# yamrom/smash-paper

Hardware: AMD Instinct MI355X
Metric: reads/sec mapped+binned (hg19, 150 bp) at 1/2/4/8 MI355X; bit-exact bin counts (higher is better)
Workload: dtype u8/u64 (integer); 1 GPU; C3 hg19-shaped, 50 M x 150 bp SMASH reads per rank (25 M pairs, one run in batches), sample_bins/50000; genome=hg19, index_words=packed (SA / ISA hints, DESIGN section 3), genome_bp=3095693983, text_N=6191388016, pairs_per_rank=25000000, read_len=150, batch_pairs=12500000, bins=50000, parallelism=single GPU

## Files before the change

smash-paper_amd/csrc/keyset.hpp:

```cpp
#pragma once

namespace smash {
namespace {

constexpr int kRefShift = 40;
constexpr uint64_t kRefPub = 1ull << 39;
struct KeyRef {
  const uint64_t *w;
  uint32_t nk;
  uint64_t lo;
};

__device__ bool same_key(const uint64_t *rec, const KeyRef &k) {
  if (rec[0] != k.lo || rec[1] != k.nk) return false;
  for (uint32_t i = 0; i < k.nk; ++i)
    if (rec[2 + i] != k.w[i]) return false;
  return true;
}

__device__ bool same_key(const KeyRef &a, const KeyRef &b) {
  if (a.lo != b.lo || a.nk != b.nk) return false;
  for (uint32_t i = 0; i < a.nk; ++i)
    if (a.w[i] != b.w[i]) return false;
  return true;
}

__device__ inline void key_hashes(const uint64_t *w, uint32_t nk, uint64_t mask, uint64_t &hh,
                                  uint64_t &hl) {
  hh = 0x9E3779B97F4A7C15ull;
  hl = 0xD1B54A32D192ED03ull;
  for (uint32_t i = 0; i < nk; ++i) {
    const uint64_t x = w[i];
    hh = mix64(hh ^ x) + 0x632BE59BD9B4E019ull;
    hl = mix64(hl + x * 0x9E3779B97F4A7C15ull) ^ (hl >> 29);
  }
  hh = (mix64(hh ^ uint64_t(nk)) & mask) | 1;
  hl = (mix64(hl + uint64_t(nk)) & mask) | 1;
}

__host__ __device__ __forceinline__ uint64_t key_home(uint64_t hi, uint64_t mask) {
  return (hi ^ (hi >> 31)) & mask;
}

__device__ __forceinline__ uint32_t wave_incl(uint32_t v, uint32_t &total) {
  const uint32_t lane = threadIdx.x & 63;
#pragma unroll
  for (int d = 1; d < 64; d <<= 1) {
    const uint32_t y = __shfl_up(v, d, 64);
    if (lane >= uint32_t(d)) v += y;
  }
  total = __shfl(v, 63, 64);
  return v;
}

__device__ __forceinline__ uint32_t wave_word_owner(uint32_t incl, uint32_t t, uint32_t &before) {
  uint32_t l = 0;
#pragma unroll
  for (uint32_t step = 32; step; step >>= 1)
    if (uint32_t(__shfl(int(incl), int(l + step - 1), 64)) <= t) l += step;
  l = l < 63u ? l : 63u;
  const uint32_t prev = uint32_t(__shfl(int(incl), int((l + 63u) & 63u), 64));
  before = l ? prev : 0u;
  return l;
}

constexpr uint32_t kDecGroups = 4;

__device__ __forceinline__ void wave_fill_records(uint64_t *arena, uint64_t off, uint32_t incl,
                                                  uint32_t total, bool ok, uint64_t lo, uint32_t m,
                                                  const uint64_t *src) {
  const uint32_t lane = threadIdx.x & 63;
  const uint64_t srcv = reinterpret_cast<uint64_t>(src);
  for (uint32_t t0 = 0; t0 < total; t0 += 64) {
    const uint32_t t = t0 + lane;
    uint32_t before;
    const uint32_t l = wave_word_owner(incl, t, before);
    const uint32_t r = t - before;
    const bool lok = __shfl(int(ok), int(l), 64) != 0;
    const uint64_t loff = __shfl(off, int(l), 64), llo = __shfl(lo, int(l), 64);
    const uint32_t lm = uint32_t(__shfl(int(m), int(l), 64));
    const uint64_t *ls = reinterpret_cast<const uint64_t *>(__shfl(srcv, int(l), 64));
    if (t < total && lok) arena[loff + r] = r == 0 ? llo : r == 1 ? uint64_t(lm) : ls[r - 2];
  }
}

constexpr uint64_t kSlotOld = ~0ull, kSlotNone = ~0ull - 1;
constexpr uint64_t kSlotIns = 1ull << 62;

struct PairKeys {
  static constexpr bool kMarks = true;
  const int32_t *nk;
  const uint64_t *hash;
  HitRows hits;
  uint8_t *contest;
  __device__ __forceinline__ int32_t count(uint64_t q) const { return nk[q]; }
  __device__ __forceinline__ KeyRef key(uint64_t q, uint64_t *hi = nullptr) const {
    if (hi) *hi = hash[2 * q];
    const int32_t k = nk[q];
    return KeyRef{hits.row(q, k), uint32_t(k), hash[2 * q + 1]};
  }
};

struct RecvKeys {
  static constexpr bool kMarks = false;
  const uint64_t *recv, *words, *base;
  int world;
  uint64_t hmask;
  __device__ __forceinline__ int32_t count(uint64_t j) const {
    return int32_t(recv[kHdrWords * j] >> 40);
  }
  __device__ __forceinline__ KeyRef key(uint64_t j, uint64_t *hi = nullptr) const {
    int r = 0;
    while (r + 1 < world && j >= base[r + 1]) ++r;
    const uint64_t nw = recv[kHdrWords * j];
    KeyRef k{words + base[65 + r] + (nw & kHdrOffMask), uint32_t(nw >> 40), 0};
    uint64_t h = 0;
    key_hashes(k.w, k.nk, hmask, h, k.lo);
    if (hi) *hi = h;
    return k;
  }
};

template <class Src>
__device__ __forceinline__ uint64_t claim_key(const Src &src, uint64_t j, uint64_t *table,
                                              uint64_t mask, const uint64_t *arena,
                                              uint64_t epoch, int32_t &err) {
  uint64_t hi = 0;
  const KeyRef me = src.key(j, &hi);
  const unsigned long long mine = (epoch << kRefShift) | (j + 1);
  uint64_t res = kSlotNone;
  uint64_t i = key_home(hi, mask);
  uint32_t waits = 0;
  for (uint64_t probe = 0; probe <= mask;) {
    unsigned long long *sh = reinterpret_cast<unsigned long long *>(&table[2 * i]);
    unsigned long long *sr = sh + 1;
    unsigned long long cur = __hip_atomic_load(sh, __ATOMIC_RELAXED, __HIP_MEMORY_SCOPE_AGENT);
    if (cur == 0) {
      const unsigned long long prev = atomicCAS(sh, 0ull, (unsigned long long)hi);
      if (prev == 0) {
        __hip_atomic_store(sr, mine, __ATOMIC_RELAXED, __HIP_MEMORY_SCOPE_AGENT);
        res = Src::kMarks ? i | kSlotIns : i;
        break;
      }
      cur = prev;
    }
    if (cur == hi) {
      const unsigned long long ref =
          __hip_atomic_load(sr, __ATOMIC_RELAXED, __HIP_MEMORY_SCOPE_AGENT);
      if (ref == 0) {
        if (++waits > (1u << 22)) {
          err = SMASH_ERR_UNSUPPORTED;
          break;
        }
        continue;
      }
      if (ref & kRefPub) {
        if ((ref >> kRefShift) != epoch &&
            same_key(arena + ((ref & (kRefPub - 1)) - 1), me)) {
          res = kSlotOld;
          break;
        }
      } else if ((ref >> kRefShift) == epoch) {
        const uint64_t j2 = (ref & (kRefPub - 1)) - 1;
        if (same_key(me, src.key(j2))) {
          if constexpr (Src::kMarks) src.contest[j2] = 1;
          atomicMin(sr, mine);
          res = i;
          break;
        }
      }
    }
    ++probe;
    i = (i + 1) & mask;
  }
  if (res == kSlotNone && err == 0) err = SMASH_ERR_NOMEM;
  return res;
}

template <class Src, class Item>
__device__ __forceinline__ bool decide_keys(const Src &src, uint64_t n, uint64_t *table,
                                            uint64_t *arena, uint64_t arena_cap,
                                            unsigned long long *arena_top, uint64_t epoch,
                                            const uint64_t *__restrict__ slot_of, Item item) {
  const uint64_t stride = uint64_t(gridDim.x) * blockDim.x;
  bool full = false;
  const uint32_t lane = threadIdx.x & 63;
  for (uint64_t c0 = (uint64_t(blockIdx.x) * blockDim.x + (threadIdx.x & ~63u)) * kDecGroups;
       c0 < n; c0 += stride * kDecGroups) {
    bool wins[kDecGroups];
    uint32_t needs[kDecGroups], incls[kDecGroups], tots[kDecGroups];
    uint32_t sum = 0;
#pragma unroll
    for (uint32_t g = 0; g < kDecGroups; ++g) {
      const uint64_t j = c0 + 64 * g + lane;
      const int32_t m = j < n ? src.count(j) : -1;
      bool win = false;
      if (m >= 0) {
        const uint64_t sl = slot_of[j];
        bool sole = false;
        if constexpr (Src::kMarks) sole = sl < kSlotNone && (sl & kSlotIns) && !src.contest[j];
        if (sole) {
          win = true;
        } else if (sl < kSlotNone) {
          const unsigned long long ref = __hip_atomic_load(
              reinterpret_cast<unsigned long long *>(&table[2 * (sl & ~kSlotIns) + 1]),
              __ATOMIC_RELAXED, __HIP_MEMORY_SCOPE_AGENT);
          win = ref == ((epoch << kRefShift) | (j + 1));
        }
      }
      wins[g] = win;
      needs[g] = win ? 2u + uint32_t(m) : 0u;
      incls[g] = wave_incl(needs[g], tots[g]);
      sum += tots[g];
    }
    unsigned long long wbase = 0;
    if (lane == 63 && sum) wbase = atomicAdd(arena_top, (unsigned long long)sum);
    wbase = __shfl(wbase, 63, 64);
#pragma unroll
    for (uint32_t g = 0; g < kDecGroups; ++g) {
      const uint64_t j = c0 + 64 * g + lane;
      const bool win = wins[g];
      const uint32_t need = needs[g], incl = incls[g], total = tots[g];
      const uint64_t off = uint64_t(wbase) + incl - need;
      wbase += total;
      const bool ok = win && off + need <= arena_cap;
      KeyRef me{nullptr, 0u, 0ull};
      if (win) me = src.key(j);
      wave_fill_records(arena, off, incl, total, ok, me.lo, me.nk, me.w);
      if (win) {
        if (!ok) {
          full = true;
        } else {
          __hip_atomic_store(
              reinterpret_cast<unsigned long long *>(&table[2 * (slot_of[j] & ~kSlotIns) + 1]),
              (unsigned long long)((epoch << kRefShift) | kRefPub | (off + 1)), __ATOMIC_RELAXED,
              __HIP_MEMORY_SCOPE_AGENT);
        }
      }
      if (j < n) item(j, win);
    }
  }
  return full;
}

__global__ void k_dedup_claim(const int32_t *__restrict__ nk, const uint64_t *__restrict__ hash,
                              HitRows hits, uint64_t n,
                              uint64_t *table, uint64_t mask, const uint64_t *arena,
                              uint64_t epoch, uint64_t *slot_of, uint8_t *contest,
                              unsigned long long *stats) {
  SMASH_BESIDE_SEARCH();
  const PairKeys src{nk, hash, hits, contest};
  const uint64_t stride = uint64_t(gridDim.x) * blockDim.x;
  int32_t err = 0;
  for (uint64_t q = uint64_t(blockIdx.x) * blockDim.x + threadIdx.x; q < n; q += stride)
    if (nk[q] >= 0) slot_of[q] = claim_key(src, q, table, mask, arena, epoch, err);
  if (err) atomicCAS(&stats[S_ERR], 0ull, (unsigned long long)(unsigned)err);
}

__global__ void k_dedup_decide(const int32_t *__restrict__ nk, const uint64_t *__restrict__ hash,
                               HitRows hits,
                               const uint32_t *__restrict__ nmajor,
                               const int64_t *__restrict__ chrom_off, uint64_t n,
                               uint64_t *table, uint64_t *arena, uint64_t arena_cap,
                               unsigned long long *arena_top, uint64_t epoch,
                               const uint64_t *__restrict__ slot_of,
                               const uint8_t *__restrict__ contest, uint8_t *keep,
                               uint32_t *cnt, int64_t *lp, unsigned long long *stats) {
  SMASH_BESIDE_SEARCH();
  const PairKeys src{nk, hash, hits, const_cast<uint8_t *>(contest)};
  unsigned long long kp = 0, dp = 0;
  const bool full = decide_keys(
      src, n, table, arena, arena_cap, arena_top, epoch, slot_of,
      [&](uint64_t q, bool win) __attribute__((always_inline)) {
        const int32_t m = nk[q];
        if (m >= 0) {
          ++kp;
          dp += win ? 0 : 1;
        }
        keep[q] = win ? 1 : 0;
        const uint32_t c = win ? nmajor[q] : 0;
        cnt[q] = c;
        int64_t last = -1;
        if (c) {
          const uint64_t *h = hits.row(q, m);
          for (int32_t j = m - 1; j >= 0; --j)
            if (chrom_off[uint32_t(h[j] >> 48)] >= 0) {
              last = int64_t(h[j] & 0xFFFFFFFFFFFFull);
              break;
            }
        }
        lp[q] = last;
      });
  wave_stats(stats, S_KEYPAIRS, kp, S_DUPEPAIRS, dp, full ? SMASH_ERR_NOMEM : 0);
}

__global__ void k_owner_claim(const uint64_t *recv, const uint64_t *words, const uint64_t *base,
                              int world, uint64_t n, uint64_t *table, uint64_t mask,
                              const uint64_t *arena, uint64_t epoch, uint64_t *slot_of,
                              unsigned long long *stats, uint64_t hmask) {
  const RecvKeys src{recv, words, base, world, hmask};
  const uint64_t stride = uint64_t(gridDim.x) * blockDim.x;
  int32_t err = 0;
  for (uint64_t j = uint64_t(blockIdx.x) * blockDim.x + threadIdx.x; j < n; j += stride)
    slot_of[j] = claim_key(src, j, table, mask, arena, epoch, err);
  if (err) atomicCAS(&stats[S_ERR], 0ull, (unsigned long long)(unsigned)err);
}

__global__ void k_owner_decide(const uint64_t *recv, const uint64_t *words, const uint64_t *base,
                               int world, uint64_t n, uint64_t *table, uint64_t *arena,
                               uint64_t arena_cap, unsigned long long *arena_top, uint64_t epoch,
                               const uint64_t *__restrict__ slot_of, uint8_t *flags,
                               unsigned long long *stats, uint64_t hmask) {
  const RecvKeys src{recv, words, base, world, hmask};
  const bool full = decide_keys(src, n, table, arena, arena_cap, arena_top, epoch, slot_of,
                                [&](uint64_t j, bool win) __attribute__((always_inline)) {
                                  flags[j] = win ? 1 : 0;
                                });
  if (full) atomicCAS(&stats[S_ERR], 0ull, (unsigned long long)(unsigned)SMASH_ERR_NOMEM);
}

}
}

static void key_set_geometry(uint64_t keys, uint64_t max_pairs, uint64_t *slots,
                             uint64_t *arena_words) {
  const uint64_t cap = 2 * std::max<uint64_t>(keys, max_pairs);
  uint64_t pw = 1;
  while (pw < cap) pw <<= 1;
  *slots = pw;
  *arena_words = std::min<uint64_t>(16 * std::max<uint64_t>(keys, max_pairs) + (1u << 20),
                                    smash::kRefPub - 2);
}

static uint64_t next_epoch(smash_pipeline *p) {
  p->epoch = p->epoch % ((1ull << (64 - smash::kRefShift)) - 1) + 1;
  return p->epoch;
}

__global__ void k_rehash(const uint64_t *__restrict__ old, uint64_t old_slots, uint64_t *nt,
                         uint64_t mask) {
  const uint64_t stride = uint64_t(gridDim.x) * blockDim.x;
  for (uint64_t i = uint64_t(blockIdx.x) * blockDim.x + threadIdx.x; i < old_slots; i += stride) {
    const uint64_t hi = old[2 * i];
    if (!hi) continue;
    uint64_t j = smash::key_home(hi, mask);
    for (uint64_t probe = 0; probe <= mask; ++probe, j = (j + 1) & mask) {
      unsigned long long *sh = reinterpret_cast<unsigned long long *>(&nt[2 * j]);
      if (atomicCAS(sh, 0ull, (unsigned long long)hi) == 0ull) {
        nt[2 * j + 1] = old[2 * i + 1];
        break;
      }
    }
  }
}
```

smash-paper_amd/csrc/pipeline.hip:

```cpp
#include <hipcub/hipcub.hpp>

#include <algorithm>
#include <cstdlib>
#include <cstring>

#include "common.hpp"
#include "mam_device.hpp"

namespace {
constexpr int kB = 256;
constexpr unsigned kPostBlocks = 64;
constexpr unsigned kPostThreads = kPostBlocks * kB;
enum Stat { S_PAIRS, S_KEYPAIRS, S_DUPEPAIRS, S_POS, S_DUPS, S_KEPT, S_MATCHES, S_ERR, S_N };
constexpr uint32_t kStatStride = 16, kStatStripes = 16, kStatWords = kStatStride * kStatStripes;
constexpr uint32_t kHdrWords = 1;
constexpr uint64_t kHdrOffMask = (uint64_t(1) << 40) - 1;
static_assert(kHdrWords == SMASH_EXPORT_HDR_WORDS, "smash_gpu.h's export header");
}

#define SMASH_BESIDE_SEARCH() __builtin_amdgcn_s_setprio(2)

struct smash_pipeline {
  const smash_index *ix = nullptr;
  int device = 0;
  uint32_t read_len = 0, min_len = 20, slots = 0, n_contig = 0, nbins = 0;
  uint32_t stride = 0;
  int32_t min_excess = 4;
  int64_t hit_window = 10000;
  uint64_t max_pairs = 0;
  uint32_t *d_tag_off = nullptr;
  uint8_t *d_small = nullptr;
  int64_t *d_chrom_off = nullptr;
  int64_t *d_bins = nullptr;
  uint32_t *d_cell = nullptr;
  uint32_t ncell = 0, cshift = 0;
  uint32_t *d_sp_cell = nullptr;
  uint32_t sp_ncell = 0, sp_shift = 0;
  uint64_t *d_match = nullptr;
  uint32_t *d_nmatch = nullptr;
  uint64_t *d_match_s[2] = {nullptr, nullptr};
  uint32_t *d_nmatch_s[2] = {nullptr, nullptr};
  uint8_t *d_rec_s[2] = {nullptr, nullptr};
  unsigned long long *d_work_s[2] = {nullptr, nullptr};
  uint64_t rec_bytes = 0;
  bool var_len = false;
  uint16_t *d_len_s[2] = {nullptr, nullptr};
  const uint16_t *d_lens = nullptr;
  hipStream_t xs[2] = {nullptr, nullptr};
  hipEvent_t ev_in = nullptr, ev_found[2] = {nullptr, nullptr}, ev_free[2] = {nullptr, nullptr};
  hipEvent_t ev_done = nullptr;
  bool set_used[2] = {false, false};
  bool defer_free = false;
  const uint8_t *pref_reads[2] = {nullptr, nullptr};
  uint64_t pref_n[2] = {0, 0};
  bool searched[2] = {false, false};
  int set = 1;
  int32_t *d_nk = nullptr;
  uint32_t *d_nmajor = nullptr;
  uint64_t *d_hits = nullptr;
  uint64_t *d_hhead = nullptr;
  uint64_t *d_hash = nullptr;
  uint8_t *d_keep = nullptr;
  uint64_t *d_slot = nullptr;
  uint8_t *d_contest = nullptr;
  uint64_t *d_tsum = nullptr;
  int64_t *d_tlast = nullptr;
  bool cnt_ready = false;
  bool reads_resident = false;
  uint64_t *d_bcnt = nullptr, *d_boff = nullptr;
  void *d_scan_temp = nullptr;
  size_t scan_temp_bytes = 0;
  uint64_t *d_oslot = nullptr;
  uint64_t oslot_cap = 0;
  uint64_t *d_table = nullptr;
  uint64_t table_mask = 0;
  uint64_t *d_arena = nullptr;
  uint64_t arena_cap = 0;
  unsigned long long *d_arena_top = nullptr;
  uint64_t keys_bound = 0;
  uint64_t epoch = 0;
  uint32_t *d_posoff = nullptr;
  uint32_t *d_cnt = nullptr;
  int64_t *d_pos0 = nullptr, *d_abs = nullptr;
  int64_t *d_prev = nullptr;
  int64_t *d_lp = nullptr, *d_lps = nullptr;
  uint32_t bin_flush = 0x8000;
  uint32_t *d_binpart = nullptr;
  bool bin_lds = true;
  bool pos_dirty = false;
  unsigned long long *d_stats = nullptr;
  uint32_t *d_fb = nullptr;
  uint32_t *d_l16 = nullptr;
  uint8_t *d_post_ws = nullptr;
  uint64_t hash_mask = ~0ull;
  bool post_fast = false;
  bool mhint = false;
  uint32_t post_cap = 0;
  uint32_t *d_send_q = nullptr;
  unsigned long long *d_owner = nullptr;
  uint64_t *d_send_hdr = nullptr;
  uint64_t *d_send_words = nullptr;
  uint64_t send_words_cap = 0;
  uint64_t *d_recv_base = nullptr;
  unsigned long long *h_owner = nullptr;
  uint64_t *h_recv_base = nullptr;
  hipEvent_t ev_base = nullptr;
  uint64_t n_pairs = 0, n_export = 0;
  hipStream_t last = nullptr;
  void *feed = nullptr;
  void (*feed_free)(void *) = nullptr;
  bool prof = false;
  std::vector<hipEvent_t> ev;
  uint64_t n_ev = 0, prof_reads = 0;
};

namespace smash {
namespace {

struct PostCfg {
  const uint64_t *startpos, *sizes;
  uint32_t n_seq, L, slots;
  const uint32_t *tag_off;
  const uint8_t *small;
  const int64_t *chrom_off;
  const uint8_t *map;
  uint64_t map_bytes;
  int32_t min_excess;
  int64_t window;
  uint32_t fast_cap;
  uint64_t hash_mask;
  const uint32_t *sp_cell;
  uint32_t sp_shift, sp_ncell;
  bool mhint;
  const uint16_t *lens;
};

constexpr uint64_t kRefMask = kPkPosMask;

constexpr uint32_t kHitHead = 16;
struct HitRows {
  uint64_t *head, *full;
  uint32_t slots;
  __device__ __forceinline__ uint64_t *row(uint64_t q, int32_t nk) const {
    return nk <= int32_t(kHitHead) ? head + q * kHitHead : full + q * 2 * uint64_t(slots);
  }
};

struct Aln {
  int64_t pos, qpos;
  uint32_t seq;
  uint16_t prefix, len, suffix;
  uint8_t rc, pad;
};

struct Hit {
  int64_t pos;
  uint32_t tid, qstart, qend;
  int32_t L0, R0;
  int64_t qkey;
  uint8_t rc;
};

__device__ inline bool merge_less(const Aln &a, const Aln &b) {
  if (a.rc != b.rc) return a.rc < b.rc;
  if (a.seq != b.seq) return a.seq < b.seq;
  if (a.pos != b.pos) return a.pos < b.pos;
  return a.prefix < b.prefix;
}

__device__ inline unsigned mapb(const PostCfg &c, uint64_t at) {
  return at < c.map_bytes ? c.map[at] : 0u;
}

template <bool VAR>
__device__ int mate_hits(const PostCfg &c, const uint64_t *m, uint32_t n,
                         Hit *hits, Aln *a, int32_t &err, uint32_t Lm) {
  int na = 0;
  const uint32_t L = VAR ? Lm : c.L;
  for (uint32_t k = 0; k < n; ++k) {
    const uint64_t w = m[k];
    const uint64_t ref = w & (c.mhint ? kRefMask : 0xFFFFFFFFFFFFull);
    const uint32_t q = uint32_t((w >> 48) & 0xFF), len = uint32_t(w >> 56);
    uint32_t lo = 0, hi = c.n_seq;
    while (lo < hi) {
      const uint32_t mid = (lo + hi) >> 1;
      if (c.startpos[mid] <= ref) lo = mid + 1; else hi = mid;
    }
    const uint32_t si = lo - 1;
    const uint64_t rcpos = ref - q;
    int64_t pos = int64_t(rcpos - c.startpos[si]);
    const uint32_t extra = L - len - q;
    Aln x;
    x.qpos = q;
    x.len = uint16_t(len);
    if (si & 1) {
      x.seq = si - 1;
      pos = int64_t(c.sizes[si - 1] - uint64_t(pos)) - int64_t(L);
      x.prefix = uint16_t(extra);
      x.suffix = uint16_t(q);
      x.rc = 1;
    } else {
      x.seq = si;
      x.prefix = uint16_t(q);
      x.suffix = uint16_t(extra);
      x.rc = 0;
    }
    x.pos = pos;
    if (pos >= 0) a[na++] = x;
  }
  for (int i = 1; i < na; ++i) {
    Aln t = a[i];
    int j = i - 1;
    while (j >= 0 && merge_less(t, a[j])) { a[j + 1] = a[j]; --j; }
    a[j + 1] = t;
  }
  int nh = 0;
  int g0 = 0;
  for (int i = 0; i < na; ++i) {
    const bool endg = (i + 1 == na) || a[i + 1].pos != a[i].pos ||
                      a[i + 1].seq != a[i].seq || a[i + 1].rc != a[i].rc;
    if (!endg) continue;
    Hit h;
    h.tid = a[i].seq >> 1;
    h.rc = a[i].rc;
    h.pos = a[i].pos;
    h.qstart = a[g0].prefix;
    h.qend = L - a[i].suffix;
    int64_t qmin = a[g0].qpos;
    for (int k = g0 + 1; k <= i; ++k) qmin = a[k].qpos < qmin ? a[k].qpos : qmin;
    h.qkey = qmin;
    const uint32_t abspos = c.tag_off[h.tid] + uint32_t(h.pos + 1);
    const bool small = c.small[h.tid] != 0;
    for (int k = g0; k <= i; ++k) {
      const uint32_t cnt = a[k].len;
      const uint32_t li = abspos + uint32_t(a[k].prefix) + cnt - 1;
      const uint32_t ri = abspos + uint32_t(a[k].prefix) - 1;
      const unsigned lm = mapb(c, 2 + uint64_t(li) * 2);
      const unsigned left = lm ? lm - 1 : 255;
      const unsigned rm = mapb(c, 2 + uint64_t(ri) * 2 + 1);
      const unsigned right = rm ? rm : 255;
      if (k == g0) { h.L0 = int32_t(left); h.R0 = int32_t(right); }
      if (!small && err == 0) {
        if (left > cnt) err = SMASH_ERR_TAG_LEFT;
        else if (right > cnt) err = SMASH_ERR_TAG_RIGHT;
      }
    }
    int j = nh - 1;
    while (j >= 0 && (h.qkey < hits[j].qkey || (h.qkey == hits[j].qkey && h.rc < hits[j].rc))) {
      hits[j + 1] = hits[j];
      --j;
    }
    hits[j + 1] = h;
    ++nh;
    g0 = i + 1;
  }
  return nh;
}

__device__ inline uint64_t mix64(uint64_t z) {
  z ^= z >> 33; z *= 0xff51afd7ed558ccdull;
  z ^= z >> 33; z *= 0xc4ceb9fe1a85ec53ull;
  z ^= z >> 33;
  return z;
}

__host__ __device__ inline uint64_t post_ws_bytes(uint32_t slots) {
  return (uint64_t(slots) * sizeof(Aln) + 2ull * slots * sizeof(Hit) + 15) & ~uint64_t(15);
}

template <bool VAR>
__device__ __noinline__ void post_pair(const PostCfg &c, const uint64_t *__restrict__ match,
                                       const uint32_t *__restrict__ nmatch, uint64_t q,
                                       int32_t *nk_out, uint32_t *nmajor_out,
                                       HitRows hits_out, uint64_t *hash_out, int32_t &err,
                                       unsigned long long &nm, uint8_t *ws) {
  {
    Aln *a = reinterpret_cast<Aln *>(ws);
    Hit *h1 = reinterpret_cast<Hit *>(ws + uint64_t(c.slots) * sizeof(Aln));
    Hit *h2 = h1 + c.slots;
    const uint32_t n1 = nmatch[2 * q], n2 = nmatch[2 * q + 1];
    nm = n1 + n2;
    const uint32_t L1 = VAR ? c.lens[2 * q] : 0u, L2 = VAR ? c.lens[2 * q + 1] : 0u;
    const int k1 = mate_hits<VAR>(c, match + (2 * q) * c.slots, n1 < c.slots ? n1 : c.slots, h1, a,
                                  err, L1);
    const int k2 = mate_hits<VAR>(c, match + (2 * q + 1) * c.slots, n2 < c.slots ? n2 : c.slots, h2,
                                  a, err, L2);
    if (n1 > c.slots || n2 > c.slots) err = SMASH_ERR_UNSUPPORTED;
    int m1 = 0, m2 = 0;
    for (int i = 0; i < k1; ++i) {
      const int mx = h1[i].L0 > h1[i].R0 ? h1[i].L0 : h1[i].R0;
      if (int(h1[i].qend) - int(h1[i].qstart) - mx >= c.min_excess) h1[m1++] = h1[i];
    }
    for (int i = 0; i < k2; ++i) {
      const int mx = h2[i].L0 > h2[i].R0 ? h2[i].L0 : h2[i].R0;
      if (int(h2[i].qend) - int(h2[i].qstart) - mx >= c.min_excess) h2[m2++] = h2[i];
    }
    uint64_t *ho = hits_out.full + q * (2 * uint64_t(c.slots));
    int32_t nk = -1;
    uint32_t nmaj = 0;
    uint64_t hh = 0x9E3779B97F4A7C15ull, hl = 0xD1B54A32D192ED03ull;
    if (m1 > 0 || m2 > 0) {
      nk = 0;
      auto put = [&](uint32_t tid, int64_t pos) {
        ho[nk++] = (uint64_t(tid) << 48) | (uint64_t(pos) & 0xFFFFFFFFFFFFull);
        const uint64_t w = (uint64_t(tid) << 48) ^ uint64_t(pos);
        hh = mix64(hh ^ w) + 0x632BE59BD9B4E019ull;
        hl = mix64(hl + w * 0x9E3779B97F4A7C15ull) ^ (hl >> 29);
        if (c.chrom_off[tid] >= 0) ++nmaj;
      };
      for (int i = 0; i < m1; ++i) put(h1[i].tid, h1[i].pos);
      for (int b = 0; b < m2; ++b) {
        bool close = false;
        for (int i = 0; i < m1; ++i) {
          int64_t d = h1[i].pos - h2[b].pos;
          d = d < 0 ? -d : d;
          if (h1[i].tid == h2[b].tid && d < c.window) { close = true; break; }
        }
        if (!close) put(h2[b].tid, h2[b].pos);
      }
      hh = (mix64(hh ^ uint64_t(nk)) & c.hash_mask) | 1;
      hl = (mix64(hl + uint64_t(nk)) & c.hash_mask) | 1;
      if (nk <= int32_t(kHitHead))
        for (int32_t i = 0; i < nk; ++i) hits_out.head[q * kHitHead + i] = ho[i];
    }
    nk_out[q] = nk;
    nmajor_out[q] = nmaj;
    hash_out[2 * q] = hh;
    hash_out[2 * q + 1] = hl;
  }
}

__device__ __forceinline__ unsigned long long wave_sum(unsigned long long v) {
#pragma unroll
  for (int d = 32; d >= 1; d >>= 1) v += __shfl_xor(v, d, 64);
  return v;
}

__device__ __forceinline__ unsigned long long *stat_row(unsigned long long *stats) {
  const uint32_t w = blockIdx.x * (blockDim.x / 64) + threadIdx.x / 64;
  return stats + kStatStride * (w % kStatStripes);
}

__device__ __forceinline__ void wave_stats(unsigned long long *stats, int ia,
                                           unsigned long long a, int ib, unsigned long long b,
                                           int32_t err) {
  a = wave_sum(a);
  b = wave_sum(b);
  unsigned long long *row = stat_row(stats);
  if ((threadIdx.x & 63) == 0) {
    if (a) atomicAdd(&row[ia], a);
    if (b) atomicAdd(&row[ib], b);
  }
  if (err) atomicCAS(&stats[S_ERR], 0ull, (unsigned long long)(unsigned)err);
}

__device__ __forceinline__ void post_stats(unsigned long long nm, unsigned long long np,
                                           int32_t err, unsigned long long *stats) {
  wave_stats(stats, S_MATCHES, nm, S_PAIRS, np, err);
}

template <bool VAR>
__global__ __launch_bounds__(kB) void k_post(PostCfg c, const uint64_t *__restrict__ match,
                                             const uint32_t *__restrict__ nmatch,
                                             uint64_t n_pairs, const uint32_t *list,
                                             const uint32_t *n_list, int32_t *nk_out,
                                             uint32_t *nmajor_out, HitRows hits_out,
                                             uint64_t *hash_out, unsigned long long *stats,
                                             uint8_t *ws) {
  SMASH_BESIDE_SEARCH();
  int32_t err = 0;
  unsigned long long nm = 0, np = 0;
  const uint64_t t = uint64_t(blockIdx.x) * blockDim.x + threadIdx.x;
  uint8_t *my = ws + t * post_ws_bytes(c.slots);
  const uint64_t n = list ? *n_list : n_pairs;
  for (uint64_t i = t; i < n; i += uint64_t(gridDim.x) * blockDim.x) {
    unsigned long long m = 0;
    post_pair<VAR>(c, match, nmatch, list ? list[i] : i, nk_out, nmajor_out, hits_out, hash_out, err,
              m, my);
    nm += m;
    ++np;
  }
  post_stats(nm, np, err, stats);
}

__device__ __forceinline__ uint32_t zero_byte(uint32_t w) {
  const uint32_t z = (w - 0x01010101u) & ~w & 0x80808080u;
  return z ? uint32_t(__builtin_ctz(z)) >> 3 : 4u;
}

__global__ __launch_bounds__(kB) void k_row_lens(const uint8_t *__restrict__ rows, uint64_t stride,
                                                 uint32_t max_len, uint64_t n, bool wide,
                                                 uint16_t *__restrict__ lens) {
  SMASH_BESIDE_SEARCH();
  const uint64_t r = uint64_t(blockIdx.x) * blockDim.x + threadIdx.x;
  if (r >= n) return;
  const uint8_t *row = rows + r * stride;
  uint32_t i = 0;
  bool found = false;
  if (wide) {
    const uint4 *v = reinterpret_cast<const uint4 *>(row);
    for (uint32_t c = 0; c < max_len && !found; c += 16) {
      const uint4 x = v[c >> 4];
      const uint32_t w[4] = {x.x, x.y, x.z, x.w};
#pragma unroll
      for (int k = 3; k >= 0; --k) {
        const uint32_t z = zero_byte(w[k]);
        if (z < 4) { found = true; i = c + 4 * uint32_t(k) + z; }
      }
    }
  } else {
    for (; i < max_len && ((reinterpret_cast<uintptr_t>(row) + i) & 3); ++i)
      if (row[i] == 0) { found = true; break; }
    for (; !found && i + 4 <= max_len; i += 4) {
      const uint32_t z = zero_byte(*reinterpret_cast<const uint32_t *>(row + i));
      if (z < 4) { found = true; i += z; break; }
    }
    for (; !found && i < max_len; ++i)
      if (row[i] == 0) { found = true; break; }
  }
  lens[r] = uint16_t(found && i < max_len ? i : max_len);
}

constexpr int FCAP = 16;

__device__ __forceinline__ void cx(uint64_t &a, uint64_t &b) {
  const uint64_t lo = a < b ? a : b, hi = a < b ? b : a;
  a = lo;
  b = hi;
}

__device__ __forceinline__ void wave_push(uint32_t *list, uint32_t *n, bool pred, uint32_t v) {
  const uint64_t b = __ballot(pred);
  if (!b) return;
  const uint32_t lane = threadIdx.x & 63, leader = uint32_t(__builtin_ctzll(b));
  uint32_t base = 0;
  if (lane == leader) base = atomicAdd(n, uint32_t(__popcll(b)));
  base = __shfl(base, int(leader), 64);
  if (pred) list[base + uint32_t(__popcll(b & ((1ull << lane) - 1)))] = v;
}

template <int N>
__device__ __forceinline__ void sort_net2(uint64_t (&v)[N], uint32_t (&r)[N]) {
#pragma unroll
  for (int p = 1; p < N; p <<= 1)
#pragma unroll
    for (int k = p; k >= 1; k >>= 1)
#pragma unroll
      for (int j = k % p; j <= N - 1 - k; j += 2 * k)
#pragma unroll
        for (int i = 0; i < k; ++i)
          if (i + j + k < N && (i + j) / (2 * p) == (i + j + k) / (2 * p)) {
            const bool sw = v[i + j + k] < v[i + j];
            const uint64_t a = v[i + j], b = v[i + j + k];
            const uint32_t ra = r[i + j], rb = r[i + j + k];
            v[i + j] = sw ? b : a; v[i + j + k] = sw ? a : b;
            r[i + j] = sw ? rb : ra; r[i + j + k] = sw ? ra : rb;
          }
}

template <int N>
__device__ __forceinline__ void sort_net(uint64_t (&v)[N]) {
#pragma unroll
  for (int p = 1; p < N; p <<= 1)
#pragma unroll
    for (int k = p; k >= 1; k >>= 1)
#pragma unroll
      for (int j = k % p; j <= N - 1 - k; j += 2 * k)
#pragma unroll
        for (int i = 0; i < k; ++i)
          if (i + j + k < N && (i + j) / (2 * p) == (i + j + k) / (2 * p))
            cx(v[i + j], v[i + j + k]);
}

template <int CAP>
__device__ __forceinline__ void mate_fast(const PostCfg &c, const uint64_t *__restrict__ sp,
                                          const uint64_t *m, uint32_t n, uint64_t (&H)[CAP],
                                          int32_t &err, const uint32_t L) {
  uint64_t A[CAP];
  uint32_t R[CAP];
  uint64_t w[CAP];
#pragma unroll
  for (int k = 0; k < CAP; ++k) w[k] = uint32_t(k) < n ? m[k] : 0;
  const uint64_t rmask = c.mhint ? kRefMask : 0xFFFFFFFFFFFFull;
  uint32_t c0[CAP], c1[CAP];
#pragma unroll
  for (int k = 0; k < CAP; ++k) {
    uint64_t cl = (w[k] & rmask) >> c.sp_shift;
    cl = cl < c.sp_ncell ? cl : c.sp_ncell - 1;
    c0[k] = c.sp_cell[cl];
    c1[k] = c.sp_cell[cl + 1];
  }
  uint32_t lo[CAP];
  {
    uint64_t s0[CAP];
#pragma unroll
    for (int k = 0; k < CAP; ++k) s0[k] = sp[c0[k] < c.n_seq ? c0[k] : c.n_seq - 1];
#pragma unroll
    for (int k = 0; k < CAP; ++k) {
      const uint64_t ref = w[k] & rmask;
      uint32_t l = c0[k], h = c1[k];
      if (h - l <= 1) {
        l += uint32_t(l < h && s0[k] <= ref);
      } else {
        while (l < h) {
          const uint32_t mid = (l + h) >> 1;
          if (sp[mid] <= ref) l = mid + 1; else h = mid;
        }
      }
      lo[k] = uint32_t(k) < n ? l : 0u;
    }
  }
  uint64_t spi[CAP], sz[CAP];
  uint32_t toff[CAP], sml = 0;
#pragma unroll
  for (int k = 0; k < CAP; ++k) {
    const uint32_t si = lo[k] ? lo[k] - 1 : 0;
    spi[k] = sp[si];
    sz[k] = c.sizes[(si & 1) ? si - 1 : si];
    toff[k] = c.tag_off[si >> 1];
    sml |= uint32_t(c.small[si >> 1] != 0) << k;
  }
  uint32_t hint[CAP], xl[CAP], xr[CAP];
#pragma unroll
  for (int k = 0; k < CAP; ++k) {
    const uint64_t ref = w[k] & rmask;
    const uint32_t q = uint32_t((w[k] >> 48) & 0xFF), len = uint32_t(w[k] >> 56);
    const uint32_t si = lo[k] ? lo[k] - 1 : 0;
    int64_t pos = int64_t(ref - q - spi[k]);
    const uint32_t extra = L - len - q;
    const uint32_t rc = si & 1;
    if (rc) pos = int64_t(sz[k] - uint64_t(pos)) - int64_t(L);
    const uint64_t prefix = rc ? extra : q;
    const bool ok = uint32_t(k) < n && lo[k] != 0 && pos >= 0;
    A[k] = ok ? (uint64_t(rc) << 63) | (uint64_t(si >> 1) << 48) | (uint64_t(pos) << 16) |
                    (prefix << 8) | len
              : ~0ull;
    const uint64_t o = ref - spi[k];
    const uint32_t h = !c.mhint ? 0u : !rc ? uint32_t(w[k] >> 40) & 0xFFu
                       : o + len <= sz[k] ? uint32_t(w[k] >> kPkPosBits) & 0x7Fu : 0u;
    const bool edge = rc ? h >= o + len : o + h >= sz[k];
    hint[k] = h ? 0x100u | (edge ? 0u : h) : 0u;
    const uint32_t abspos = toff[k] + uint32_t(pos) + 1;
    const uint32_t bl = abspos + uint32_t(prefix) + len - 1, br = abspos + uint32_t(prefix) - 1;
    xl[k] = ok && 2 + uint64_t(bl) * 2 < c.map_bytes ? bl + 1 : 0u;
    xr[k] = ok && !hint[k] && 2 + uint64_t(br) * 2 + 1 < c.map_bytes ? br + 1 : 0u;
  }
#pragma unroll
  for (int k = 0; k < CAP; ++k) {
    const uint32_t lb = c.map[xl[k] ? uint64_t(xl[k]) * 2 : 0];
    const uint32_t rb = c.map[xr[k] ? uint64_t(xr[k]) * 2 + 1 : 0];
    const bool ok = A[k] != ~0ull;
    const uint32_t lm = xl[k] ? lb : 0u;
    const uint32_t rm = !ok ? 0u : (hint[k] & 0x100u) ? (hint[k] & 0xFFu) : xr[k] ? rb : 0u;
    R[k] = lm | (rm << 8) | (((sml >> k) & 1u) << 16);
  }
  sort_net2(A, R);
  uint32_t g_prefix = 0, g_qmin = 0;
  int32_t g_l0 = 0, g_r0 = 0;
#pragma unroll
  for (int i = 0; i < CAP; ++i) {
    const uint64_t a = A[i];
    const bool valid = a != ~0ull;
    const uint32_t rc = uint32_t(a >> 63), tid = valid ? uint32_t(a >> 48) & 0x7FFF : 0u;
    const uint32_t pos = uint32_t(a >> 16), prefix = uint32_t(a >> 8) & 0xFF, len = uint32_t(a) & 0xFF;
    const uint32_t qpos = rc ? L - len - prefix : prefix;
    const bool start = i == 0 || (A[i - 1] >> 16) != (a >> 16);
    const bool endg = i + 1 == CAP || (A[i + 1 < CAP ? i + 1 : i] >> 16) != (a >> 16);
    const uint32_t lm = R[i] & 0xFFu, rm = (R[i] >> 8) & 0xFFu;
    const int32_t left = lm ? int32_t(lm) - 1 : 255, right = rm ? int32_t(rm) : 255;
    if (start) {
      g_prefix = prefix; g_qmin = qpos; g_l0 = left; g_r0 = right;
    } else {
      g_qmin = qpos < g_qmin ? qpos : g_qmin;
    }
    if (valid && err == 0 && !((R[i] >> 16) & 1u)) {
      if (uint32_t(left) > len) err = SMASH_ERR_TAG_LEFT;
      else if (uint32_t(right) > len) err = SMASH_ERR_TAG_RIGHT;
    }
    const int32_t mx = g_l0 > g_r0 ? g_l0 : g_r0;
    const uint32_t pass = int32_t(prefix + len) - int32_t(g_prefix) - mx >= c.min_excess;
    H[i] = valid && endg ? (uint64_t(g_qmin) << 56) | (uint64_t(rc) << 55) |
                               (uint64_t(pass) << 54) | (uint64_t(tid) << 32) | pos
                         : ~0ull;
  }
  sort_net(H);
}

__device__ __forceinline__ bool hit_kept(uint64_t h) { return h != ~0ull && ((h >> 54) & 1); }

template <int CAP, bool VAR>
__global__ __launch_bounds__(kB) void k_post_fast(PostCfg c, const uint64_t *__restrict__ match,
                                                  const uint32_t *__restrict__ nmatch,
                                                  uint64_t n_pairs, const uint32_t *list,
                                                  const uint32_t *n_list, uint32_t lim,
                                                  uint32_t *up_list, uint32_t *up_n,
                                                  int32_t *nk_out, uint32_t *nmajor_out,
                                                  HitRows hits_out, uint64_t *hash_out,
                                                  unsigned long long *stats) {
  SMASH_BESIDE_SEARCH();
  const uint64_t *sp = c.startpos;
  const uint64_t n = list ? *n_list : n_pairs;
  const uint64_t stride = uint64_t(gridDim.x) * blockDim.x;
  const uint64_t t0 = uint64_t(blockIdx.x) * blockDim.x + threadIdx.x;
  int32_t err = 0;
  unsigned long long nm = 0, np = 0;
  for (uint64_t base = t0 - threadIdx.x % 64; base < n; base += stride) {
    const uint64_t i = base + threadIdx.x % 64;
    const bool in = i < n;
    const uint64_t q = in ? (list ? list[i] : i) : 0;
    const uint32_t n1 = in ? nmatch[2 * q] : 0, n2 = in ? nmatch[2 * q + 1] : 0;
    const bool over = in && (n1 > lim || n2 > lim);
    wave_push(up_list, up_n, over, uint32_t(q));
    if (in && !over) {
      nm += n1 + n2;
      ++np;
      uint64_t H1[CAP], H2[CAP];
      mate_fast<CAP>(c, sp, match + (2 * q) * c.slots, n1, H1, err, VAR ? c.lens[2 * q] : c.L);
      mate_fast<CAP>(c, sp, match + (2 * q + 1) * c.slots, n2, H2, err,
                     VAR ? c.lens[2 * q + 1] : c.L);
      uint64_t *ho = CAP <= 8 ? hits_out.head + q * kHitHead
                              : hits_out.full + q * (2 * uint64_t(c.slots));
      int32_t nk = -1;
      uint32_t nmaj = 0;
      uint64_t hh = 0x9E3779B97F4A7C15ull, hl = 0xD1B54A32D192ED03ull;
      bool any = false;
#pragma unroll
      for (int i = 0; i < CAP; ++i) any = any || hit_kept(H1[i]) || hit_kept(H2[i]);
      if (any) {
        nk = 0;
        auto put = [&](uint64_t h) {
          const uint32_t tid = uint32_t(h >> 32) & 0xFFFF;
          const int64_t pos = int64_t(uint32_t(h));
          ho[nk++] = (uint64_t(tid) << 48) | uint64_t(pos);
          const uint64_t x = (uint64_t(tid) << 48) ^ uint64_t(pos);
          hh = mix64(hh ^ x) + 0x632BE59BD9B4E019ull;
          hl = mix64(hl + x * 0x9E3779B97F4A7C15ull) ^ (hl >> 29);
          if (c.chrom_off[tid] >= 0) ++nmaj;
        };
#pragma unroll
        for (int i = 0; i < CAP; ++i)
          if (hit_kept(H1[i])) put(H1[i]);
#pragma unroll
        for (int b = 0; b < CAP; ++b) {
          if (!hit_kept(H2[b])) continue;
          bool close = false;
#pragma unroll
          for (int i = 0; i < CAP; ++i) {
            int64_t d = int64_t(uint32_t(H1[i])) - int64_t(uint32_t(H2[b]));
            d = d < 0 ? -d : d;
            close |= hit_kept(H1[i]) && ((H1[i] >> 32) & 0xFFFF) == ((H2[b] >> 32) & 0xFFFF) &&
                     d < c.window;
          }
          if (!close) put(H2[b]);
        }
        hh = (mix64(hh ^ uint64_t(nk)) & c.hash_mask) | 1;
        hl = (mix64(hl + uint64_t(nk)) & c.hash_mask) | 1;
        if (CAP > 8 && nk <= int32_t(kHitHead))
          for (int32_t i = 0; i < nk; ++i) hits_out.head[q * kHitHead + i] = ho[i];
      }
      nk_out[q] = nk;
      nmajor_out[q] = nmaj;
      hash_out[2 * q] = hh;
      hash_out[2 * q + 1] = hl;
    }
  }
  post_stats(nm, np, err, stats);
}

constexpr uint32_t kScanPer = 16, kScanTile = 64 * kScanPer;

__device__ __forceinline__ int64_t last_valid(int64_t a, int64_t b) { return b >= 0 ? b : a; }

__device__ __forceinline__ void wave_scan(uint64_t &s, int64_t &l) {
  const uint32_t lane = threadIdx.x & 63;
#pragma unroll
  for (int d = 1; d < 64; d <<= 1) {
    const uint64_t ys = __shfl_up(s, d, 64);
    const int64_t yl = __shfl_up(l, d, 64);
    if (lane >= uint32_t(d)) {
      s += ys;
      l = last_valid(yl, l);
    }
  }
}

__device__ __forceinline__ void scan_run(const uint32_t *__restrict__ cnt,
                                         const int64_t *__restrict__ lp, uint64_t q0, uint64_t n,
                                         uint32_t (&c)[kScanPer], int64_t (&v)[kScanPer]) {
  if (q0 + kScanPer <= n) {
    const uint4 *cv = reinterpret_cast<const uint4 *>(cnt + q0);
    const longlong2 *lv = reinterpret_cast<const longlong2 *>(lp + q0);
#pragma unroll
    for (uint32_t k = 0; k < kScanPer / 4; ++k) {
      const uint4 x = cv[k];
      c[4 * k] = x.x; c[4 * k + 1] = x.y; c[4 * k + 2] = x.z; c[4 * k + 3] = x.w;
    }
#pragma unroll
    for (uint32_t k = 0; k < kScanPer / 2; ++k) {
      const longlong2 y = lv[k];
      v[2 * k] = y.x; v[2 * k + 1] = y.y;
    }
  } else {
#pragma unroll
    for (uint32_t k = 0; k < kScanPer; ++k) {
      const bool ok = q0 + k < n;
      c[k] = ok ? cnt[q0 + k] : 0;
      v[k] = ok ? lp[q0 + k] : -1;
    }
  }
}

__global__ void k_scan_tiles(const uint32_t *__restrict__ cnt, const int64_t *__restrict__ lp,
                             uint64_t n, uint64_t *tsum, int64_t *tlast) {
  SMASH_BESIDE_SEARCH();
  const uint64_t t = (uint64_t(blockIdx.x) * blockDim.x + threadIdx.x) / 64;
  const uint64_t q0 = t * kScanTile + uint64_t(threadIdx.x & 63) * kScanPer;
  uint64_t s = 0;
  int64_t l = -1;
  if (t * kScanTile < n) {
    uint32_t c[kScanPer];
    int64_t v[kScanPer];
    scan_run(cnt, lp, q0, n, c, v);
#pragma unroll
    for (uint32_t k = 0; k < kScanPer; ++k) {
      s += c[k];
      l = last_valid(l, v[k]);
    }
  }
  wave_scan(s, l);
  if ((threadIdx.x & 63) == 63 && t * kScanTile < n) {
    tsum[t] = s;
    tlast[t] = l;
  }
}

constexpr uint32_t kTopBlk = 16;
__global__ void k_scan_top(uint64_t *tsum, int64_t *tlast, uint64_t ntile) {
  SMASH_BESIDE_SEARCH();
  const uint32_t lane = threadIdx.x & 63;
  const uint64_t per = (ntile + 63) / 64;
  const uint64_t a = lane * per < ntile ? lane * per : ntile;
  const uint64_t b = a + per < ntile ? a + per : ntile;
  uint64_t s = 0;
  int64_t l = -1;
  for (uint64_t t0 = a; t0 < b; t0 += kTopBlk) {
    uint64_t ts[kTopBlk];
    int64_t tl[kTopBlk];
#pragma unroll
    for (uint32_t k = 0; k < kTopBlk; ++k) {
      const bool in = t0 + k < b;
      ts[k] = in ? tsum[t0 + k] : 0;
      tl[k] = in ? tlast[t0 + k] : -1;
    }
#pragma unroll
    for (uint32_t k = 0; k < kTopBlk; ++k) {
      s += ts[k];
      l = last_valid(l, tl[k]);
    }
  }
  uint64_t is = s;
  int64_t il = l;
  wave_scan(is, il);
  uint64_t es = __shfl_up(is, 1, 64);
  int64_t el = __shfl_up(il, 1, 64);
  if (lane == 0) { es = 0; el = -1; }
  for (uint64_t t0 = a; t0 < b; t0 += kTopBlk) {
    uint64_t ts[kTopBlk];
    int64_t tl[kTopBlk];
#pragma unroll
    for (uint32_t k = 0; k < kTopBlk; ++k) {
      const bool in = t0 + k < b;
      ts[k] = in ? tsum[t0 + k] : 0;
      tl[k] = in ? tlast[t0 + k] : -1;
    }
#pragma unroll
    for (uint32_t k = 0; k < kTopBlk; ++k) {
      if (t0 + k < b) {
        tsum[t0 + k] = es;
        tlast[t0 + k] = el;
      }
      es += ts[k];
      el = last_valid(el, tl[k]);
    }
  }
}

__global__ void k_scan_apply(const uint32_t *__restrict__ cnt, const int64_t *__restrict__ lp,
                             uint64_t n, const uint64_t *__restrict__ tsum,
                             const int64_t *__restrict__ tlast, uint32_t *posoff, int64_t *lps) {
  SMASH_BESIDE_SEARCH();
  const uint64_t t = (uint64_t(blockIdx.x) * blockDim.x + threadIdx.x) / 64;
  const uint64_t q0 = t * kScanTile + uint64_t(threadIdx.x & 63) * kScanPer;
  const bool live = t * kScanTile < n;
  uint32_t c[kScanPer];
  int64_t v[kScanPer];
  uint64_t s = 0;
  int64_t l = -1;
  scan_run(cnt, lp, q0, live ? n : 0, c, v);
#pragma unroll
  for (uint32_t k = 0; k < kScanPer; ++k) {
    s += c[k];
    l = last_valid(l, v[k]);
  }
  uint64_t is = s;
  int64_t il = l;
  wave_scan(is, il);
  uint64_t es = __shfl_up(is, 1, 64);
  int64_t el = __shfl_up(il, 1, 64);
  if ((threadIdx.x & 63) == 0) { es = 0; el = -1; }
  if (!live) return;
  es += tsum[t];
  el = last_valid(tlast[t], el);
  if (q0 + kScanPer <= n) {
    uint32_t po[kScanPer];
    int64_t lo[kScanPer];
#pragma unroll
    for (uint32_t k = 0; k < kScanPer; ++k) {
      es += c[k];
      el = last_valid(el, v[k]);
      po[k] = uint32_t(es);
      lo[k] = el;
    }
    __builtin_memcpy(posoff + q0 + 1, po, sizeof(po));
    __builtin_memcpy(lps + q0, lo, sizeof(lo));
    return;
  }
#pragma unroll
  for (uint32_t k = 0; k < kScanPer; ++k) {
    if (q0 + k >= n) break;
    es += c[k];
    el = last_valid(el, v[k]);
    posoff[q0 + k + 1] = uint32_t(es);
    lps[q0 + k] = el;
  }
}

__global__ void k_emit(const uint8_t *keep, const int32_t *nk,
                       HitRows hits, const uint32_t *off, uint64_t n,
                       const int64_t *chrom_off, int64_t *pos0, int64_t *absp) {
  const uint64_t q = uint64_t(blockIdx.x) * blockDim.x + threadIdx.x;
  if (q >= n || !keep[q]) return;
  const uint64_t *h = hits.row(q, nk[q]);
  uint64_t o = off[q];
  for (int32_t i = 0; i < nk[q]; ++i) {
    const uint32_t tid = uint32_t(h[i] >> 48);
    const int64_t p = int64_t(h[i] & 0xFFFFFFFFFFFFull);
    const int64_t co = chrom_off[tid];
    if (co < 0) continue;
    pos0[o] = p;
    absp[o] = p + co;
    ++o;
  }
}

__device__ __forceinline__ uint32_t bin_of(int64_t a, const int64_t *__restrict__ bins,
                                           uint32_t nbins, const uint32_t *__restrict__ cell,
                                           uint32_t ncell, uint32_t cshift) {
  uint32_t lo = 0, hi = nbins;
  if (cell) {
    uint64_t c = a < 0 ? 0 : uint64_t(a) >> cshift;
    c = c < ncell ? c : ncell - 1;
    lo = cell[c];
    hi = cell[c + 1];
  }
  while (lo < hi) {
    const uint32_t mid = (lo + hi) >> 1;
    if (a < bins[mid]) hi = mid; else lo = mid + 1;
  }
  return lo == 0 ? nbins - 1 : lo - 1;
}

__global__ __launch_bounds__(kB) void k_bin(const int64_t *__restrict__ pos0,
                                            const int64_t *__restrict__ absp,
                                            const uint32_t *npos_p, const int64_t *prev_p,
                                            const int64_t *__restrict__ bins, uint32_t nbins,
                                            const uint32_t *__restrict__ cell, uint32_t ncell,
                                            uint32_t cshift, unsigned long long *counts,
                                            unsigned long long *stats) {
  const uint64_t n = *npos_p;
  const int64_t prev0 = *prev_p;
  unsigned long long d = 0, k = 0, t = 0;
  const uint64_t stride = uint64_t(gridDim.x) * blockDim.x;
  for (uint64_t i = uint64_t(blockIdx.x) * blockDim.x + threadIdx.x; i < n; i += stride) {
    const int64_t p = pos0[i];
    const int64_t pr = i ? pos0[i - 1] : prev0;
    ++t;
    if (pr >= 0 && pr == p) { ++d; continue; }
    atomicAdd(&counts[bin_of(absp[i], bins, nbins, cell, ncell, cshift)], 1ull);
    ++k;
  }
  __shared__ unsigned long long sd, sk, st;
  if (threadIdx.x == 0) { sd = 0; sk = 0; st = 0; }
  __syncthreads();
  if (t) { atomicAdd(&st, t); atomicAdd(&sd, d); atomicAdd(&sk, k); }
  __syncthreads();
  if (threadIdx.x == 0 && st) {
    atomicAdd(&stats[S_POS], st);
    atomicAdd(&stats[S_DUPS], sd);
    atomicAdd(&stats[S_KEPT], sk);
  }
}

__global__ void k_count_last(const uint8_t *keep, const uint32_t *nmajor, const int32_t *nk,
                             HitRows hits, const int64_t *chrom_off,
                             uint64_t n, uint32_t *cnt, int64_t *lp) {
  const uint64_t q = uint64_t(blockIdx.x) * blockDim.x + threadIdx.x;
  if (q >= n) return;
  const uint32_t c = keep[q] ? nmajor[q] : 0;
  cnt[q] = c;
  int64_t last = -1;
  if (c) {
    const uint64_t *h = hits.row(q, nk[q]);
    for (int32_t i = nk[q] - 1; i >= 0; --i)
      if (chrom_off[uint32_t(h[i] >> 48)] >= 0) {
        last = int64_t(h[i] & 0xFFFFFFFFFFFFull);
        break;
      }
  }
  lp[q] = last;
}

__global__ __launch_bounds__(kB) void k_emit_bin(
    const uint8_t *__restrict__ keep, const int32_t *__restrict__ nk,
    HitRows hits, const int64_t *__restrict__ chrom_off,
    const int64_t *__restrict__ lps, uint64_t n, const int64_t *prev_p,
    const int64_t *__restrict__ bins, uint32_t nbins, const uint32_t *__restrict__ cell,
    uint32_t ncell, uint32_t cshift, unsigned long long *counts, unsigned long long *stats) {
  SMASH_BESIDE_SEARCH();
  const int64_t prev0 = *prev_p;
  unsigned long long d = 0, k = 0, t = 0;
  const uint64_t stride = uint64_t(gridDim.x) * blockDim.x;
  for (uint64_t q = uint64_t(blockIdx.x) * blockDim.x + threadIdx.x; q < n; q += stride) {
    if (!keep[q]) continue;
    const int32_t m = nk[q];
    if (m <= 0) continue;
    int64_t prev = q ? lps[q - 1] : -1;
    if (prev < 0) prev = prev0;
    const uint64_t *h = hits.row(q, m);
    for (int32_t i = 0; i < m; ++i) {
      const uint64_t w = h[i];
      const int64_t co = chrom_off[uint32_t(w >> 48)];
      if (co < 0) continue;
      const int64_t p = int64_t(w & 0xFFFFFFFFFFFFull);
      ++t;
      if (prev >= 0 && prev == p) {
        ++d;
      } else {
        atomicAdd(&counts[bin_of(p + co, bins, nbins, cell, ncell, cshift)], 1ull);
        ++k;
      }
      prev = p;
    }
  }
  wave_stats(stats, S_POS, t, S_DUPS, d, 0);
  wave_stats(stats, S_KEPT, k, S_KEPT, 0, 0);
}

constexpr uint32_t kBinPart = 77824;
constexpr uint32_t kBinPartsMax = 4;
constexpr uint32_t kBinBlocks = 256;
inline uint32_t bin_parts(uint32_t nbins) { return (nbins + kBinPart - 1) / kBinPart; }
inline uint32_t bin_part_size(uint32_t nbins) {
  const uint32_t np = bin_parts(nbins);
  return np ? (nbins + np - 1) / np : 1;
}
__global__ __launch_bounds__(1024) void k_emit_bin_lds(
    const uint8_t *__restrict__ keep, const int32_t *__restrict__ nk,
    HitRows hits, const int64_t *__restrict__ chrom_off,
    const int64_t *__restrict__ lps, uint64_t n, const int64_t *prev_p,
    const int64_t *__restrict__ bins, uint32_t nbins, const uint32_t *__restrict__ cell,
    uint32_t ncell, uint32_t cshift, unsigned long long *counts, unsigned long long *stats,
    uint32_t part, uint32_t flush, uint32_t *binpart) {
  __shared__ uint32_t hc[kBinPart / 2];
  const uint32_t b0 = blockIdx.y * part;
  const uint32_t b1 = b0 + part < nbins ? b0 + part : nbins;
  for (uint32_t i = threadIdx.x; i < (part + 1) / 2; i += blockDim.x) hc[i] = 0;
  __syncthreads();
  const int64_t prev0 = *prev_p;
  unsigned long long d = 0, k = 0, t = 0;
  const uint64_t stride = uint64_t(gridDim.x) * blockDim.x;
  struct Ahead {
    uint32_t kp;
    int32_t m;
    int64_t lp;
    uint4 h0, h1;
  };
  auto fetch = [&](uint64_t x) {
    Ahead a{0u, 0, -1, make_uint4(0, 0, 0, 0), make_uint4(0, 0, 0, 0)};
    if (x < n) {
      a.kp = keep[x];
      a.m = nk[x];
      a.lp = x ? lps[x - 1] : -1;
      const uint4 *r = reinterpret_cast<const uint4 *>(hits.head + x * kHitHead);
      a.h0 = r[0];
      a.h1 = r[1];
    }
    return a;
  };
  uint64_t q = uint64_t(blockIdx.x) * blockDim.x + threadIdx.x;
  Ahead cur = fetch(q);
  for (; q < n; q += stride) {
    const Ahead nxt = fetch(q + stride);
    const int32_t m = cur.kp ? cur.m : 0;
    int64_t prev = cur.lp < 0 ? prev0 : cur.lp;
    const uint64_t *h = hits.row(q, cur.m);
    const int32_t pre = cur.m <= int32_t(kHitHead) ? 4 : 0;
    for (int32_t i = 0; i < m; ++i) {
      const uint4 &hv = i < 2 ? cur.h0 : cur.h1;
      const uint64_t w = i >= pre ? h[i]
                                : (i & 1) ? (uint64_t(hv.w) << 32 | hv.z) : (uint64_t(hv.y) << 32 | hv.x);
      const int64_t co = chrom_off[uint32_t(w >> 48)];
      if (co < 0) continue;
      const int64_t p = int64_t(w & 0xFFFFFFFFFFFFull);
      ++t;
      if (prev >= 0 && prev == p) {
        ++d;
      } else {
        const uint32_t b = bin_of(p + co, bins, nbins, cell, ncell, cshift);
        if (b >= b0 && b < b1) {
          const uint32_t sh = 16 * ((b - b0) & 1);
          const uint32_t old = atomicAdd(&hc[(b - b0) >> 1], 1u << sh);
          if (((old >> sh) & 0xFFFFu) == flush - 1) {
            atomicSub(&hc[(b - b0) >> 1], flush << sh);
            atomicAdd(&counts[b], (unsigned long long)flush);
          }
        }
        ++k;
      }
      prev = p;
    }
    cur = nxt;
  }
  __shared__ unsigned long long sd, sk, st;
  if (threadIdx.x == 0) { sd = 0; sk = 0; st = 0; }
  __syncthreads();
  if (blockIdx.y == 0 && t) { atomicAdd(&st, t); atomicAdd(&sd, d); atomicAdd(&sk, k); }
  __syncthreads();
  if (threadIdx.x == 0 && st) {
    atomicAdd(&stats[S_POS], st);
    atomicAdd(&stats[S_DUPS], sd);
    atomicAdd(&stats[S_KEPT], sk);
  }
  uint32_t *out = binpart + uint64_t(blockIdx.x) * nbins;
  for (uint32_t i = threadIdx.x; b0 + i < b1; i += blockDim.x)
    out[b0 + i] = (hc[i >> 1] >> (16 * (i & 1))) & 0xFFFFu;
}

__global__ void k_bin_reduce(const uint32_t *__restrict__ binpart, uint32_t blocks, uint32_t nbins,
                             unsigned long long *counts) {
  for (uint32_t b = blockIdx.x * blockDim.x + threadIdx.x; b < nbins; b += gridDim.x * blockDim.x) {
    unsigned long long t = 0;
    for (uint32_t k = 0; k < blocks; ++k) t += binpart[uint64_t(k) * nbins + b];
    if (t) atomicAdd(&counts[b], t);
  }
}

__global__ void k_tail_lps(const uint32_t *npos_p, const int64_t *lps_last, int64_t *prev,
                           int64_t *tail) {
  const uint32_t c = *npos_p;
  const int64_t last = c ? *lps_last : -1;
  if (tail) { tail[0] = int64_t(c); tail[1] = last; }
  if (prev && c) prev[0] = last;
}

__global__ void k_reset_prev(int64_t *prev) {
  prev[0] = -1;
  prev[1] = -1;
}

hipError_t ensure_positions(smash_pipeline *p) {
  if (p->d_pos0 && p->d_abs) return hipSuccess;
  const uint64_t n = p->max_pairs * 2 * p->slots;
  hipError_t e = p->d_pos0 ? hipSuccess : hipMalloc(reinterpret_cast<void **>(&p->d_pos0), 8 * n);
  if (e == hipSuccess) e = hipMalloc(reinterpret_cast<void **>(&p->d_abs), 8 * n);
  if (e != hipSuccess) {
    (void)hipFree(p->d_pos0);
    p->d_pos0 = nullptr;
    p->d_abs = nullptr;
  }
  return e;
}

int check_pipe(smash_pipeline *p, uint64_t n_pairs) {
  if (!p) { set_error("null pipeline"); return SMASH_ERR_ARG; }
  if (n_pairs > p->max_pairs) {
    set_error("batch larger than cfg.max_pairs");
    return SMASH_ERR_ARG;
  }
  return SMASH_OK;
}

PostCfg post_cfg(const smash_pipeline *p) {
  PostCfg c;
  c.startpos = p->ix->d_startpos;
  c.sizes = p->ix->d_sizes;
  c.n_seq = p->ix->n_seq;
  c.L = p->read_len;
  c.slots = p->slots;
  c.tag_off = p->d_tag_off;
  c.small = p->d_small;
  c.chrom_off = p->d_chrom_off;
  c.map = p->ix->d_map;
  c.map_bytes = p->ix->map_bytes;
  c.min_excess = p->min_excess;
  c.window = p->hit_window;
  c.fast_cap = p->post_cap;
  c.hash_mask = p->hash_mask;
  c.sp_cell = p->d_sp_cell;
  c.sp_shift = p->sp_shift;
  c.sp_ncell = p->sp_ncell;
  c.mhint = p->mhint;
  c.lens = p->d_lens;
  return c;
}

HitRows hit_rows(const smash_pipeline *p) { return HitRows{p->d_hhead, p->d_hits, p->slots}; }

}
}

#include "keyset.hpp"

using namespace smash;

extern "C" uint64_t smash_pipeline_max_batch(uint32_t read_len, uint32_t min_len) {
  if (read_len == 0 || read_len > 255 || min_len < 2 || read_len < min_len) return 0;
  const uint64_t slots = read_len - min_len + 1;
  return ((1ull << 32) - 1) / (2 * slots);
}

extern "C" int smash_pipeline_create(const smash_index *ix,
                                     const smash_pipeline_cfg *cfg,
                                     smash_pipeline **out) {
  if (!ix || !cfg || !out || cfg->read_len == 0 || cfg->read_len > 255 ||
      cfg->min_len < 2 || cfg->read_len < cfg->min_len || cfg->max_pairs == 0 ||
      cfg->max_pairs > smash_pipeline_max_batch(cfg->read_len, cfg->min_len) ||
      cfg->n_contig * 2 != ix->n_seq ||
      !cfg->h_tag_offsets || !cfg->h_small_chr || !cfg->h_chrom_off ||
      !cfg->h_bin_starts || cfg->nbins == 0) {
    set_error("smash_pipeline_create: bad configuration");
    return SMASH_ERR_ARG;
  }
  if (cfg->read_stride && cfg->read_stride != cfg->read_len &&
      cfg->read_stride != smash_read_stride(cfg->read_len)) {
    set_error("smash_pipeline_create: read_stride must be 0, read_len or smash_read_stride(read_len)");
    return SMASH_ERR_ARG;
  }
  if (!ix->rcref) {
    set_error("smash_pipeline_create: the count chain needs the -rcref text layout");
    return SMASH_ERR_ARG;
  }
  if (!ix->d_map) {
    set_error("smash_pipeline_create: index has no map.bin");
    return SMASH_ERR_ARG;
  }
  auto *p = new smash_pipeline;
  try {
    SMASH_HIPX(hipSetDevice(ix->device));
    p->ix = ix;
    p->device = ix->device;
    p->read_len = cfg->read_len;
    p->stride = cfg->read_stride ? cfg->read_stride : cfg->read_len;
    p->min_len = cfg->min_len;
    p->slots = cfg->read_len - cfg->min_len + 1;
    p->n_contig = cfg->n_contig;
    p->nbins = cfg->nbins;
    p->min_excess = cfg->min_excess;
    p->hit_window = cfg->hit_window;
    p->max_pairs = cfg->max_pairs;
    const uint64_t P = cfg->max_pairs;
    p->d_tag_off = dalloc<uint32_t>(p->n_contig);
    p->d_small = dalloc<uint8_t>(p->n_contig);
    p->d_chrom_off = dalloc<int64_t>(p->n_contig);
    p->d_bins = dalloc<int64_t>(p->nbins);
    SMASH_HIPX(hipMemcpy(p->d_tag_off, cfg->h_tag_offsets, 4 * p->n_contig, hipMemcpyHostToDevice));
    {
      const char *mh = getenv("SMASH_MAP_HINT");
      bool ok = !(mh && mh[0] == '0') && ix->pos_mask == kPkPosMask && ix->rcref && ix->d_map &&
                ix->map_own;
      uint64_t off = 0;
      for (uint32_t t = 0; ok && t < p->n_contig; ++t) {
        ok = cfg->h_tag_offsets[t] == off;
        off += ix->sizes[2 * t];
      }
      p->mhint = ok;
    }
    SMASH_HIPX(hipMemcpy(p->d_small, cfg->h_small_chr, p->n_contig, hipMemcpyHostToDevice));
    SMASH_HIPX(hipMemcpy(p->d_chrom_off, cfg->h_chrom_off, 8 * p->n_contig, hipMemcpyHostToDevice));
    SMASH_HIPX(hipMemcpy(p->d_bins, cfg->h_bin_starts, 8 * p->nbins, hipMemcpyHostToDevice));
    {
      const int64_t *b = cfg->h_bin_starts;
      bool ok = b[0] >= 0;
      for (uint32_t k = 1; k < p->nbins && ok; ++k) ok = b[k] >= b[k - 1];
      if (ok) {
        const uint64_t top = uint64_t(b[p->nbins - 1]);
        uint32_t sh = 10;
        while ((top >> sh) + 2 > (1u << 18)) ++sh;
        p->cshift = sh;
        p->ncell = uint32_t((top >> sh) + 2);
        std::vector<uint32_t> cell(p->ncell + 1);
        uint32_t r = 0;
        for (uint32_t c = 0; c < p->ncell; ++c) {
          const int64_t x = int64_t(uint64_t(c) << sh);
          while (r < p->nbins && b[r] <= x) ++r;
          cell[c] = r;
        }
        cell[p->ncell] = p->nbins;
        p->d_cell = dalloc<uint32_t>(p->ncell + 1);
        SMASH_HIPX(hipMemcpy(p->d_cell, cell.data(), 4 * (p->ncell + 1), hipMemcpyHostToDevice));
      }
    }
    {
      const std::vector<uint64_t> &sp = ix->startpos;
      const uint64_t top = ix->N;
      uint32_t sh = 8;
      while ((top >> sh) + 2 > (1u << 16)) ++sh;
      p->sp_shift = sh;
      p->sp_ncell = uint32_t((top >> sh) + 2);
      std::vector<uint32_t> cell(p->sp_ncell + 1);
      uint32_t r = 0;
      for (uint32_t c = 0; c < p->sp_ncell; ++c) {
        const uint64_t x = uint64_t(c) << sh;
        while (r < sp.size() && sp[r] <= x) ++r;
        cell[c] = r;
      }
      cell[p->sp_ncell] = uint32_t(sp.size());
      p->d_sp_cell = dalloc<uint32_t>(p->sp_ncell + 1);
      SMASH_HIPX(hipMemcpy(p->d_sp_cell, cell.data(), 4 * (p->sp_ncell + 1), hipMemcpyHostToDevice));
    }
    p->rec_bytes = search_rec_bytes(2 * P, p->read_len);
    int search_prio = 0;
    if (const char *e = getenv("SMASH_SEARCH_PRIO")) {
      int least = 0, greatest = 0;
      SMASH_HIPX(hipDeviceGetStreamPriorityRange(&least, &greatest));
      if (!strcmp(e, "high")) search_prio = greatest;
      else if (!strcmp(e, "low")) search_prio = least;
    }
    for (int k = 0; k < 2; ++k) {
      p->d_match_s[k] = dalloc<uint64_t>(2 * P * p->slots);
      p->d_nmatch_s[k] = dalloc<uint32_t>(2 * P);
      p->d_work_s[k] = dalloc<unsigned long long>(1);
      if (search_prio) {
        SMASH_HIPX(hipStreamCreateWithPriority(&p->xs[k], hipStreamNonBlocking, search_prio));
      } else {
        SMASH_HIPX(hipStreamCreateWithFlags(&p->xs[k], hipStreamNonBlocking));
      }
      SMASH_HIPX(hipEventCreateWithFlags(&p->ev_found[k], hipEventDisableTiming));
      SMASH_HIPX(hipEventCreateWithFlags(&p->ev_free[k], hipEventDisableTiming));
    }
    SMASH_HIPX(hipEventCreateWithFlags(&p->ev_in, hipEventDisableTiming));
    SMASH_HIPX(hipEventCreateWithFlags(&p->ev_done, hipEventDisableTiming));
    SMASH_HIPX(hipEventRecord(p->ev_done, nullptr));
    SMASH_HIPX(hipEventSynchronize(p->ev_done));
    p->d_match = p->d_match_s[0];
    p->d_nmatch = p->d_nmatch_s[0];
    p->d_nk = dalloc<int32_t>(P);
    p->d_nmajor = dalloc<uint32_t>(P);
    p->d_hits = dalloc<uint64_t>(P * 2 * p->slots);
    p->d_hhead = dalloc<uint64_t>(P * smash::kHitHead);
    p->d_hash = dalloc<uint64_t>(2 * P);
    p->d_keep = dalloc<uint8_t>(P);
    {
      const uint64_t nb = 64 * ((P + kB - 1) / kB);
      p->d_bcnt = dalloc<uint64_t>(nb);
      p->d_boff = dalloc<uint64_t>(nb);
      SMASH_HIPX(hipcub::DeviceScan::ExclusiveSum(nullptr, p->scan_temp_bytes, p->d_bcnt,
                                                  p->d_boff, nb));
      p->d_scan_temp = dalloc<uint8_t>(p->scan_temp_bytes);
    }
    p->d_posoff = dalloc<uint32_t>(P + 1);
    p->d_cnt = dalloc<uint32_t>(P);
    uint64_t pw = 0;
    key_set_geometry(cfg->dedup_capacity, P, &pw, &p->arena_cap);
    p->table_mask = pw - 1;
    p->d_table = dalloc<uint64_t>(2 * pw);
    SMASH_HIPX(hipMemset(p->d_table, 0, 16 * pw));
    p->d_arena = dalloc<uint64_t>(p->arena_cap);
    p->d_arena_top = dalloc<unsigned long long>(1);
    SMASH_HIPX(hipMemset(p->d_arena_top, 0, 8));
    p->d_prev = dalloc<int64_t>(2);
    p->d_lp = dalloc<int64_t>(P);
    p->d_lps = dalloc<int64_t>(P);
    {
      const char *l = getenv("SMASH_BIN_LDS");
      p->bin_lds = !(l && l[0] == '0') && bin_parts(p->nbins) <= kBinPartsMax;
      if (p->bin_lds) p->d_binpart = dalloc<uint32_t>(uint64_t(kBinBlocks) * p->nbins);
      const char *fl = getenv("SMASH_BIN_FLUSH");
      const unsigned long f = fl ? std::strtoul(fl, nullptr, 10) : 0;
      if (f >= 2 && f <= 0x8000 && !(f & (f - 1))) p->bin_flush = uint32_t(f);
    }
    int64_t init[2] = {-1, -1};
    SMASH_HIPX(hipMemcpy(p->d_prev, init, 16, hipMemcpyHostToDevice));
    p->d_stats = dalloc<unsigned long long>(kStatWords);
    SMASH_HIPX(hipMemset(p->d_stats, 0, 8 * kStatWords));
    p->d_slot = dalloc<uint64_t>(P);
    p->d_contest = dalloc<uint8_t>(P);
    p->d_tsum = dalloc<uint64_t>(P / kScanTile + 1);
    p->d_tlast = dalloc<int64_t>(P / kScanTile + 1);
    p->d_send_q = dalloc<uint32_t>(P);
    p->d_fb = dalloc<uint32_t>(P + 1);
    p->d_l16 = dalloc<uint32_t>(P + 1);
    p->d_post_ws = dalloc<uint8_t>(uint64_t(kPostThreads) * post_ws_bytes(p->slots));
    {
      bool ok = p->n_contig < 0x7FFF;
      for (uint64_t z : ix->sizes) ok = ok && z < (1ull << 31);
      const char *e = getenv("SMASH_POST_LEGACY");
      p->post_fast = ok && !(e && *e && *e != '0');
      const char *pc = getenv("SMASH_POST_CAP");
      const uint32_t cap = pc && *pc ? uint32_t(atoi(pc)) : uint32_t(FCAP);
      p->post_cap = std::min<uint32_t>({cap, uint32_t(FCAP), p->slots});
    }
    if (const char *hb = getenv("SMASH_KEY_HASH_BITS")) {
      const int b = atoi(hb);
      if (b > 0 && b < 64) p->hash_mask = (1ull << b) - 1;
    }
    p->d_owner = dalloc<unsigned long long>(4 * 64);
    p->d_send_hdr = dalloc<uint64_t>(uint64_t(kHdrWords) * P);
    p->d_recv_base = dalloc<uint64_t>(2 * 65);
    SMASH_HIPX(hipHostMalloc(reinterpret_cast<void **>(&p->h_owner), 8 * 256, hipHostMallocDefault));
    SMASH_HIPX(hipHostMalloc(reinterpret_cast<void **>(&p->h_recv_base), 8 * 2 * 65,
                             hipHostMallocDefault));
    SMASH_HIPX(hipEventCreateWithFlags(&p->ev_base, hipEventDisableTiming));
    SMASH_HIPX(hipMemset(p->d_posoff, 0, 4));
  } catch (hip_failure &f) {
    set_error(f.what);
    smash_pipeline_free(p);
    return SMASH_ERR_NOMEM;
  }
  *out = p;
  return SMASH_OK;
}

namespace smash {
uint32_t pipe_read_len(const smash_pipeline *p) { return p->read_len; }
uint32_t pipe_stride(const smash_pipeline *p) { return p->stride; }
bool pipe_var_len(const smash_pipeline *p) { return p->var_len; }
uint64_t pipe_max_pairs(const smash_pipeline *p) { return p->max_pairs; }
int pipe_device(const smash_pipeline *p) { return p->device; }
void *&pipe_feed(smash_pipeline *p, void (*freer)(void *)) {
  p->feed_free = freer;
  return p->feed;
}
}

extern "C" void smash_pipeline_free(smash_pipeline *p) {
  if (!p) return;
  (void)hipSetDevice(p->device);
  if (p->feed && p->feed_free) p->feed_free(p->feed);
  for (hipEvent_t e : p->ev) (void)hipEventDestroy(e);
  for (int k = 0; k < 2; ++k) {
    if (p->xs[k]) {
      (void)hipStreamSynchronize(p->xs[k]);
      (void)hipStreamDestroy(p->xs[k]);
    }
    if (p->ev_found[k]) (void)hipEventDestroy(p->ev_found[k]);
    if (p->ev_free[k]) (void)hipEventDestroy(p->ev_free[k]);
    for (void *q : {(void *)p->d_match_s[k], (void *)p->d_nmatch_s[k], (void *)p->d_rec_s[k],
                    (void *)p->d_work_s[k], (void *)p->d_len_s[k]})
      dfree(q);
  }
  if (p->ev_in) (void)hipEventDestroy(p->ev_in);
  if (p->ev_done) (void)hipEventDestroy(p->ev_done);
  if (p->ev_base) (void)hipEventDestroy(p->ev_base);
  if (p->h_owner) (void)hipHostFree(p->h_owner);
  if (p->h_recv_base) (void)hipHostFree(p->h_recv_base);
  for (void *q : {(void *)p->d_tag_off, (void *)p->d_small, (void *)p->d_chrom_off,
                  (void *)p->d_bins, (void *)p->d_cell, (void *)p->d_sp_cell,
                  (void *)p->d_nk, (void *)p->d_nmajor, (void *)p->d_hits, (void *)p->d_hhead,
                  (void *)p->d_hash, (void *)p->d_keep, (void *)p->d_bcnt, (void *)p->d_boff,
                  p->d_scan_temp, (void *)p->d_oslot,
                  (void *)p->d_slot, (void *)p->d_contest, (void *)p->d_tsum, (void *)p->d_tlast,
                  (void *)p->d_table,
                  (void *)p->d_posoff, (void *)p->d_cnt, (void *)p->d_pos0,
                  (void *)p->d_abs, (void *)p->d_prev, (void *)p->d_stats,
                  (void *)p->d_lp, (void *)p->d_lps, (void *)p->d_binpart,
                  (void *)p->d_send_q, (void *)p->d_owner, (void *)p->d_fb, (void *)p->d_l16,
                  (void *)p->d_post_ws, (void *)p->d_arena, (void *)p->d_arena_top,
                  (void *)p->d_send_hdr, (void *)p->d_send_words, (void *)p->d_recv_base})
    dfree(q);
  delete p;
}

static int search_into(smash_pipeline *p, int k, const uint8_t *d_reads, uint64_t n_pairs,
                       hipEvent_t in_ev) {
  hipStream_t xs = p->xs[k];
  SMASH_HIP(hipStreamWaitEvent(xs, in_ev, 0));
  if (p->prof) {
    if (2 * p->n_ev + 2 > p->ev.size()) {
      for (int q = 0; q < 64; ++q) {
        hipEvent_t e;
        SMASH_HIP(hipEventCreate(&e));
        p->ev.push_back(e);
      }
    }
    p->ix->kev[0] = p->ev[2 * p->n_ev];
    p->ix->kev[1] = p->ev[2 * p->n_ev + 1];
  }
  if ((p->var_len || !search_direct(d_reads, p->stride, p->read_len)) && !p->d_rec_s[k]) {
    SMASH_HIP(hipStreamSynchronize(xs));
    SMASH_HIP(hipMalloc(reinterpret_cast<void **>(&p->d_rec_s[k]), p->rec_bytes));
  }
  if (p->var_len) {
    if (!p->d_len_s[k]) {
      SMASH_HIP(hipStreamSynchronize(xs));
      SMASH_HIP(hipMalloc(reinterpret_cast<void **>(&p->d_len_s[k]), 2 * 2 * p->max_pairs));
    }
    if (p->set_used[k]) SMASH_HIP(hipStreamWaitEvent(xs, p->ev_free[k], 0));
    const bool wide = (reinterpret_cast<uintptr_t>(d_reads) & 15) == 0 && p->stride % 16 == 0 &&
                      p->stride >= ((p->read_len + 15u) & ~15u);
    k_row_lens<<<grid_for(2 * n_pairs, kB, 1u << 30), kB, 0, xs>>>(
        d_reads, p->stride, p->read_len, 2 * n_pairs, wide, p->d_len_s[k]);
    SMASH_HIP(hipGetLastError());
  }
  SearchWs ws{p->d_rec_s[k], p->d_rec_s[k] ? p->rec_bytes : 0, p->d_work_s[k],
              p->set_used[k] ? p->ev_free[k] : nullptr, p->mhint};
  ws.geom_len = p->read_len;
  const int rc = map_batch_impl(p->ix, SMASH_MODE_MAM, p->min_len, d_reads, p->stride,
                                p->var_len ? p->d_len_s[k] : nullptr, p->read_len, 2 * n_pairs,
                                p->d_match_s[k], p->slots, p->d_nmatch_s[k], xs, false,
                                &ws);
  p->ix->kev[0] = p->ix->kev[1] = nullptr;
  if (rc) return rc;
  if (p->prof) {
    ++p->n_ev;
    p->prof_reads += 2 * n_pairs;
  }
  SMASH_HIP(hipEventRecord(p->ev_found[k], xs));
  p->pref_reads[k] = d_reads;
  p->pref_n[k] = n_pairs;
  p->searched[k] = true;
  return SMASH_OK;
}

template <bool VAR>
static int post_stage(smash_pipeline *p, uint64_t n_pairs, hipStream_t s) {
  if (p->post_fast) {
    SMASH_HIP(hipMemsetAsync(p->d_fb, 0, 4, s));
    SMASH_HIP(hipMemsetAsync(p->d_l16, 0, 4, s));
    const PostCfg pc = post_cfg(p);
    k_post_fast<8, VAR><<<grid_for(n_pairs, kB, 1u << 30), kB, 0, s>>>(
        pc, p->d_match, p->d_nmatch, n_pairs, nullptr, nullptr, std::min(8u, p->post_cap),
        p->d_l16 + 1, p->d_l16, p->d_nk, p->d_nmajor, hit_rows(p), p->d_hash, p->d_stats);
    SMASH_HIP(hipGetLastError());
    k_post_fast<FCAP, VAR><<<grid_for(n_pairs, kB, 1024), kB, 0, s>>>(
        pc, p->d_match, p->d_nmatch, n_pairs, p->d_l16 + 1, p->d_l16, p->post_cap,
        p->d_fb + 1, p->d_fb, p->d_nk, p->d_nmajor, hit_rows(p), p->d_hash, p->d_stats);
    SMASH_HIP(hipGetLastError());
    k_post<VAR><<<kPostBlocks, kB, 0, s>>>(post_cfg(p), p->d_match, p->d_nmatch, n_pairs,
                                           p->d_fb + 1, p->d_fb, p->d_nk, p->d_nmajor, hit_rows(p),
                                           p->d_hash, p->d_stats, p->d_post_ws);
  } else {
    k_post<VAR><<<kPostBlocks, kB, 0, s>>>(post_cfg(p), p->d_match, p->d_nmatch, n_pairs, nullptr,
                                           nullptr, p->d_nk, p->d_nmajor, hit_rows(p), p->d_hash,
                                           p->d_stats, p->d_post_ws);
  }
  SMASH_HIP(hipGetLastError());
  return SMASH_OK;
}

static int phase_map_impl(smash_pipeline *p, const uint8_t *d_reads, uint64_t n_pairs,
                          hipStream_t s, hipEvent_t in_ev, const uint8_t *d_next = nullptr,
                          uint64_t n_next = 0) {
  int rc = check_pipe(p, n_pairs);
  if (rc) return rc;
  if (d_next && (rc = check_pipe(p, n_next))) return rc;
  p->last = s;
  p->n_pairs = n_pairs;
  if (!n_pairs) return SMASH_OK;
  SMASH_HIP(hipSetDevice(p->device));
  const int k = p->set ^= 1;
  p->d_match = p->d_match_s[k];
  p->d_nmatch = p->d_nmatch_s[k];
  const bool have = p->searched[k] && p->pref_reads[k] == d_reads && p->pref_n[k] == n_pairs;
  if (!in_ev && p->reads_resident) in_ev = p->ev_done;
  if (!in_ev && (!have || (d_next && n_next))) {
    in_ev = p->ev_in;
    SMASH_HIP(hipEventRecord(in_ev, s));
  }
  if (!have && (rc = search_into(p, k, d_reads, n_pairs, in_ev))) return rc;
  p->searched[k] = false;
  p->d_lens = p->var_len ? p->d_len_s[k] : nullptr;
  const bool next_have = p->searched[k ^ 1] && p->pref_reads[k ^ 1] == d_next &&
                         p->pref_n[k ^ 1] == n_next;
  if (d_next && n_next && !next_have && (rc = search_into(p, k ^ 1, d_next, n_next, in_ev)))
    return rc;
  SMASH_HIP(hipStreamWaitEvent(s, p->ev_found[k], 0));
  if ((rc = p->d_lens ? post_stage<true>(p, n_pairs, s) : post_stage<false>(p, n_pairs, s)))
    return rc;
  if (!p->defer_free)
    SMASH_HIP(hipEventRecord(p->ev_free[k], s));
  p->set_used[k] = true;
  p->cnt_ready = false;
  return SMASH_OK;
}

extern "C" int smash_phase_map(smash_pipeline *p, const uint8_t *d_reads,
                               uint64_t n_pairs, void *stream) {
  return phase_map_impl(p, d_reads, n_pairs, static_cast<hipStream_t>(stream), nullptr);
}

extern "C" int smash_phase_map_ahead(smash_pipeline *p, const uint8_t *d_reads,
                                     uint64_t n_pairs, const uint8_t *d_next, uint64_t n_next,
                                     void *stream) {
  return phase_map_impl(p, d_reads, n_pairs, static_cast<hipStream_t>(stream), nullptr, d_next,
                        n_next);
}

extern "C" int smash_phase_search_ahead(smash_pipeline *p, const uint8_t *d_reads,
                                        uint64_t n_pairs, void *stream) {
  int rc = check_pipe(p, n_pairs);
  if (rc) return rc;
  if (!n_pairs) return SMASH_OK;
  const int k = p->set;
  if (p->searched[k]) {
    set_error("smash_phase_search_ahead: the set still holds an unconsumed search");
    return SMASH_ERR_ARG;
  }
  SMASH_HIP(hipSetDevice(p->device));
  hipStream_t s = static_cast<hipStream_t>(stream);
  if (p->reads_resident) return search_into(p, k, d_reads, n_pairs, p->ev_done);
  SMASH_HIP(hipEventRecord(p->ev_in, s));
  return search_into(p, k, d_reads, n_pairs, p->ev_in);
}

static int dedup_local(smash_pipeline *p, hipStream_t s) {
  const uint64_t n = p->n_pairs;
  if (!n) return SMASH_OK;
  const uint64_t epoch = next_epoch(p);
  SMASH_HIP(hipMemsetAsync(p->d_contest, 0, n, s));
  k_dedup_claim<<<grid_for(n, kB, 8192), kB, 0, s>>>(p->d_nk, p->d_hash, hit_rows(p), n,
                                                     p->d_table, p->table_mask, p->d_arena, epoch,
                                                     p->d_slot, p->d_contest, p->d_stats);
  SMASH_HIP(hipGetLastError());
  k_dedup_decide<<<grid_for((n + kDecGroups - 1) / kDecGroups, kB, 8192), kB, 0, s>>>(
      p->d_nk, p->d_hash, hit_rows(p), p->d_nmajor, p->d_chrom_off, n, p->d_table,
      p->d_arena, p->arena_cap, p->d_arena_top, epoch, p->d_slot, p->d_contest, p->d_keep,
      p->d_cnt, p->d_lp, p->d_stats);
  SMASH_HIP(hipGetLastError());
  p->cnt_ready = true;
  return SMASH_OK;
}

extern "C" int smash_phase_positions(smash_pipeline *p, int64_t *d_tail, void *stream) {
  if (!p) return SMASH_ERR_ARG;
  hipStream_t s = static_cast<hipStream_t>(stream);
  p->last = s;
  const uint64_t n = p->n_pairs;
  if (n) {
    if (!p->cnt_ready)
      k_count_last<<<grid_for(n, kB, 1u << 30), kB, 0, s>>>(p->d_keep, p->d_nmajor, p->d_nk,
                                                           hit_rows(p), p->d_chrom_off,
                                                           n, p->d_cnt, p->d_lp);
    const uint64_t ntile = (n + kScanTile - 1) / kScanTile;
    const unsigned g = unsigned((ntile * 64 + kB - 1) / kB);
    k_scan_tiles<<<g, kB, 0, s>>>(p->d_cnt, p->d_lp, n, p->d_tsum, p->d_tlast);
    k_scan_top<<<1, 64, 0, s>>>(p->d_tsum, p->d_tlast, ntile);
    k_scan_apply<<<g, kB, 0, s>>>(p->d_cnt, p->d_lp, n, p->d_tsum, p->d_tlast, p->d_posoff,
                                  p->d_lps);
    SMASH_HIP(hipGetLastError());
    p->pos_dirty = true;
  }
  k_tail_lps<<<1, 1, 0, s>>>(p->d_posoff + n, p->d_lps + (n ? n - 1 : 0), nullptr, d_tail);
  SMASH_HIP(hipGetLastError());
  return SMASH_OK;
}

extern "C" int smash_phase_bin(smash_pipeline *p, const int64_t *d_prev,
                               uint64_t *d_counts, void *stream) {
  if (!p || !d_counts) return SMASH_ERR_ARG;
  hipStream_t s = static_cast<hipStream_t>(stream);
  p->last = s;
  const uint64_t n = p->n_pairs;
  const int64_t *prev = d_prev ? d_prev : p->d_prev;
  const uint32_t parts = bin_parts(p->nbins);
  if (n && p->bin_lds) {
    const uint32_t part = bin_part_size(p->nbins);
    const unsigned gx = unsigned(std::min<uint64_t>(kBinBlocks, (n + 1023) / 1024));
    const dim3 grid(gx, parts);
    k_emit_bin_lds<<<grid, 1024, 0, s>>>(
        p->d_keep, p->d_nk, hit_rows(p), p->d_chrom_off, p->d_lps, n, prev, p->d_bins,
        p->nbins, p->d_cell, p->ncell, p->cshift, reinterpret_cast<unsigned long long *>(d_counts),
        p->d_stats, part, p->bin_flush, p->d_binpart);
    k_bin_reduce<<<grid_for(p->nbins, kB, 1024), kB, 0, s>>>(
        p->d_binpart, gx, p->nbins, reinterpret_cast<unsigned long long *>(d_counts));
  } else if (n) {
    k_emit_bin<<<grid_for(n, kB, 8192), kB, 0, s>>>(
        p->d_keep, p->d_nk, hit_rows(p), p->d_chrom_off, p->d_lps, n, prev, p->d_bins,
        p->nbins, p->d_cell, p->ncell, p->cshift, reinterpret_cast<unsigned long long *>(d_counts),
        p->d_stats);
  }
  k_tail_lps<<<1, 1, 0, s>>>(p->d_posoff + n, p->d_lps + (n ? n - 1 : 0), p->d_prev, nullptr);
  SMASH_HIP(hipGetLastError());
  return SMASH_OK;
}

namespace smash {
int count_batch_ev(smash_pipeline *p, const uint8_t *d_reads, uint64_t n_pairs,
                   uint64_t *d_counts, hipStream_t s, hipEvent_t in_ev) {
  p->defer_free = true;
  p->keys_bound += n_pairs;
  int rc = phase_map_impl(p, d_reads, n_pairs, s, in_ev);
  p->defer_free = false;
  if (rc) return rc;
  rc = dedup_local(p, s);
  if (!rc) rc = smash_phase_positions(p, nullptr, s);
  if (!rc) rc = smash_phase_bin(p, nullptr, d_counts, s);
  if (n_pairs && hipEventRecord(p->ev_free[p->set], s) != hipSuccess && !rc) {
    set_error("hipEventRecord failed");
    rc = SMASH_ERR_HIP;
  }
  return rc;
}
}

extern "C" int smash_count_batch(smash_pipeline *p, const uint8_t *d_reads,
                                 uint64_t n_pairs, uint64_t *d_counts, void *stream) {
  return smash::count_batch_ev(p, d_reads, n_pairs, d_counts, static_cast<hipStream_t>(stream),
                               nullptr);
}

static int count_batches_impl(smash_pipeline *p, const uint8_t *d_reads, uint64_t n_pairs,
                              uint64_t batch_pairs, uint64_t *d_counts, hipStream_t s,
                              hipEvent_t ready, bool resident) {
  if (!p || (n_pairs && !d_reads) || !d_counts || batch_pairs == 0 ||
      batch_pairs > p->max_pairs) {
    set_error("smash_count_batches: bad arguments");
    return SMASH_ERR_ARG;
  }
  SMASH_HIP(hipSetDevice(p->device));
  hipEvent_t in_ev = ready ? ready : resident ? p->ev_done : nullptr;
  const bool own = !in_ev;
  int rc = SMASH_OK;
  if (own) {
    SMASH_HIP(hipEventCreateWithFlags(&in_ev, hipEventDisableTiming));
    rc = hipEventRecord(in_ev, s) == hipSuccess ? SMASH_OK : SMASH_ERR_HIP;
  }
  const uint64_t L2 = 2 * uint64_t(p->stride);
  for (uint64_t b0 = 0; rc == SMASH_OK && b0 < n_pairs; b0 += batch_pairs) {
    const uint64_t n = std::min(batch_pairs, n_pairs - b0);
    rc = smash::count_batch_ev(p, d_reads + b0 * L2, n, d_counts, s, in_ev);
  }
  if (own) (void)hipEventDestroy(in_ev);
  return rc;
}

extern "C" int smash_count_batches(smash_pipeline *p, const uint8_t *d_reads, uint64_t n_pairs,
                                   uint64_t batch_pairs, uint64_t *d_counts, void *stream) {
  return count_batches_impl(p, d_reads, n_pairs, batch_pairs, d_counts,
                            static_cast<hipStream_t>(stream), nullptr, false);
}

extern "C" int smash_count_batches_ready(smash_pipeline *p, const uint8_t *d_reads,
                                         uint64_t n_pairs, uint64_t batch_pairs,
                                         uint64_t *d_counts, void *stream, void *ready) {
  return count_batches_impl(p, d_reads, n_pairs, batch_pairs, d_counts,
                            static_cast<hipStream_t>(stream), static_cast<hipEvent_t>(ready),
                            true);
}

namespace smash {
namespace {
__device__ __forceinline__ uint64_t key_owner(uint64_t hi, int world) {
  return (hi >> 1) % uint64_t(world);
}
constexpr uint32_t kExWaves = kB / 64;

struct WaveGroup {
  uint32_t rank, wbefore;
};
__device__ __forceinline__ WaveGroup wave_owner_groups(bool act, uint32_t ow, uint32_t k,
                                                       uint32_t *s_e, uint32_t *s_w) {
  const uint32_t lane = threadIdx.x & 63;
  const uint64_t below = (1ull << lane) - 1;
  WaveGroup mine{0, 0};
  uint64_t todo = __ballot(act);
  while (todo) {
    const int leader = __builtin_ctzll(todo);
    const uint32_t o = uint32_t(__shfl(int(ow), leader, 64));
    const bool in = act && ow == o;
    const uint64_t same = __ballot(in);
    uint32_t wsum;
    const uint32_t x = wave_incl(in ? k : 0u, wsum);
    if (lane == uint32_t(leader)) {
      s_e[o] = uint32_t(__popcll(same));
      s_w[o] = wsum;
    }
    if (in) {
      mine.rank = uint32_t(__popcll(same & below));
      mine.wbefore = x - k;
    }
    todo &= ~same;
  }
  return mine;
}

__global__ __launch_bounds__(kB) void k_export_count(const int32_t *nk, const uint64_t *hash,
                                                     uint64_t n, int world, uint32_t nblk,
                                                     uint64_t *bc) {
  __shared__ uint32_t s_e[kExWaves][64], s_w[kExWaves][64];
  const uint32_t wv = threadIdx.x >> 6;
  for (uint32_t o = threadIdx.x; o < kExWaves * 64; o += blockDim.x) {
    (&s_e[0][0])[o] = 0;
    (&s_w[0][0])[o] = 0;
  }
  __syncthreads();
  const uint64_t q = uint64_t(blockIdx.x) * blockDim.x + threadIdx.x;
  const bool act = q < n && nk[q] >= 0;
  const uint32_t ow = act ? uint32_t(key_owner(hash[2 * q], world)) : 0u;
  (void)wave_owner_groups(act, ow, act ? uint32_t(nk[q]) : 0u, s_e[wv], s_w[wv]);
  __syncthreads();
  for (uint32_t o = threadIdx.x; o < uint32_t(world); o += blockDim.x) {
    uint64_t e = 0, w = 0;
    for (uint32_t v = 0; v < kExWaves; ++v) {
      e += s_e[v][o];
      w += s_w[v][o];
    }
    bc[uint64_t(o) * nblk + blockIdx.x] = (e << 32) | w;
  }
}

__global__ void k_export_totals(const uint64_t *bc, const uint64_t *boff, int world,
                                uint32_t nblk, unsigned long long *tot) {
  const uint32_t o = threadIdx.x;
  if (o >= uint32_t(world)) return;
  const uint64_t last = uint64_t(o + 1) * nblk - 1;
  const uint64_t end = boff[last] + bc[last], beg = boff[uint64_t(o) * nblk];
  tot[o] = (end >> 32) - (beg >> 32);
  tot[64 + o] = (end & 0xFFFFFFFFull) - (beg & 0xFFFFFFFFull);
}

__global__ __launch_bounds__(kB) void k_export_fill(const int32_t *nk, const uint64_t *hash,
                                                    HitRows hits,
                                                    uint64_t n, int world, uint32_t nblk,
                                                    const uint64_t *boff,
                                                    uint64_t *hdr, uint64_t *words,
                                                    uint32_t *send_q) {
  __shared__ uint32_t s_e[kExWaves][64], s_w[kExWaves][64];
  const uint32_t wv = threadIdx.x >> 6;
  for (uint32_t o = threadIdx.x; o < kExWaves * 64; o += blockDim.x) {
    (&s_e[0][0])[o] = 0;
    (&s_w[0][0])[o] = 0;
  }
  __syncthreads();
  const uint64_t q = uint64_t(blockIdx.x) * blockDim.x + threadIdx.x;
  const bool act = q < n && nk[q] >= 0;
  const uint32_t ow = act ? uint32_t(key_owner(hash[2 * q], world)) : 0u;
  const uint32_t k = act ? uint32_t(nk[q]) : 0u;
  const WaveGroup g = wave_owner_groups(act, ow, k, s_e[wv], s_w[wv]);
  __syncthreads();
  uint64_t w = 0;
  if (act) {
    uint64_t e = g.rank;
    w = g.wbefore;
    for (uint32_t v = 0; v < wv; ++v) {
      e += s_e[v][ow];
      w += s_w[v][ow];
    }
    const uint64_t bo = boff[uint64_t(ow) * nblk + blockIdx.x];
    const uint64_t seg_w = boff[uint64_t(ow) * nblk] & 0xFFFFFFFFull;
    e += bo >> 32;
    w += bo & 0xFFFFFFFFull;
    hdr[kHdrWords * e] = uint64_t(k) << 40 | (w - seg_w);
    send_q[e] = uint32_t(q);
  }
  const uint32_t lane = threadIdx.x & 63;
  uint32_t total;
  const uint32_t incl = wave_incl(k, total);
  const uint64_t row = act ? reinterpret_cast<uint64_t>(hits.row(q, int32_t(k))) : 0ull;
  for (uint32_t t0 = 0; t0 < total; t0 += 64) {
    const uint32_t t = t0 + lane;
    uint32_t before;
    const uint32_t l = wave_word_owner(incl, t, before);
    const uint64_t wl = __shfl(w, int(l), 64), rl = __shfl(row, int(l), 64);
    if (t < total) words[wl + (t - before)] = reinterpret_cast<const uint64_t *>(rl)[t - before];
  }
}

__global__ void k_import(const uint8_t *flags, const uint32_t *send_q, uint64_t n_export,
                         uint8_t *keep) {
  const uint64_t o = uint64_t(blockIdx.x) * blockDim.x + threadIdx.x;
  if (o < n_export) keep[send_q[o]] = flags[o];
}
__global__ void k_import_stats(const uint8_t *keep, const int32_t *nk, uint64_t n,
                               unsigned long long *stats) {
  const uint64_t q = uint64_t(blockIdx.x) * blockDim.x + threadIdx.x;
  const bool keyed = q < n && nk[q] >= 0;
  wave_stats(stats, S_KEYPAIRS, keyed ? 1ull : 0ull, S_DUPEPAIRS,
             keyed && !keep[q] ? 1ull : 0ull, 0);
}
}
}

extern "C" int smash_phase_export(smash_pipeline *p, int world, uint64_t global_base,
                                  int64_t *h_send_counts, int64_t *h_send_words,
                                  const uint64_t **d_send, const uint64_t **d_send_words,
                                  void *stream) {
  if (!p || world < 1 || world > 64 || !h_send_counts || !h_send_words || !d_send ||
      !d_send_words) {
    set_error("smash_phase_export: bad arguments");
    return SMASH_ERR_ARG;
  }
  hipStream_t s = static_cast<hipStream_t>(stream);
  p->last = s;
  const uint64_t n = p->n_pairs;
  const uint32_t nblk = uint32_t(std::max<uint64_t>(1, (n + kB - 1) / kB));
  SMASH_HIP(hipMemsetAsync(p->d_keep, 0, n ? n : 1, s));
  unsigned long long *cnt = p->h_owner;
  std::fill(cnt, cnt + 128, 0ull);
  if (n) {
    k_export_count<<<nblk, kB, 0, s>>>(p->d_nk, p->d_hash, n, world, nblk, p->d_bcnt);
    size_t tb = p->scan_temp_bytes;
    SMASH_HIP(hipcub::DeviceScan::ExclusiveSum(p->d_scan_temp, tb, p->d_bcnt, p->d_boff,
                                               uint64_t(world) * nblk, s));
    k_export_totals<<<1, 64, 0, s>>>(p->d_bcnt, p->d_boff, world, nblk, p->d_owner);
    SMASH_HIP(hipGetLastError());
    SMASH_HIP(hipMemcpyAsync(cnt, p->d_owner, 8 * 128, hipMemcpyDeviceToHost, s));
    SMASH_HIP(hipStreamSynchronize(s));
  }
  uint64_t tot = 0, wtot = 0;
  for (int r = 0; r < world; ++r) {
    tot += cnt[r];
    wtot += cnt[64 + r];
    h_send_counts[r] = int64_t(cnt[r]);
    h_send_words[r] = int64_t(cnt[64 + r]);
  }
  p->n_export = tot;
  if (wtot > p->send_words_cap) {
    if (p->d_send_words) SMASH_HIP(hipFree(p->d_send_words));
    p->send_words_cap = wtot + wtot / 4 + 1024;
    SMASH_HIP(hipMalloc(&p->d_send_words, 8 * p->send_words_cap));
  }
  if (n)
    k_export_fill<<<nblk, kB, 0, s>>>(p->d_nk, p->d_hash, hit_rows(p), n, world, nblk,
                                      p->d_boff, p->d_send_hdr, p->d_send_words, p->d_send_q);
  SMASH_HIP(hipGetLastError());
  *d_send = p->d_send_hdr;
  *d_send_words = p->d_send_words;
  return SMASH_OK;
}

extern "C" int smash_dedup_owner(smash_pipeline *p, const uint64_t *d_recv, uint64_t n_recv,
                                 const uint64_t *d_recv_words, const int64_t *h_recv_counts,
                                 const int64_t *h_recv_words, int world, uint8_t *d_flags,
                                 void *stream) {
  if (!p || world < 1 || world > 64 || !h_recv_counts || !h_recv_words ||
      (n_recv && (!d_recv || !d_flags))) {
    set_error("smash_dedup_owner: bad arguments");
    return SMASH_ERR_ARG;
  }
  hipStream_t s = static_cast<hipStream_t>(stream);
  SMASH_HIP(hipEventSynchronize(p->ev_base));
  uint64_t *base = p->h_recv_base;
  std::fill(base, base + 2 * 65, uint64_t(0));
  uint64_t hs = 0, ws = 0;
  for (int r = 0; r < world; ++r) {
    base[r] = hs;
    base[65 + r] = ws;
    hs += uint64_t(h_recv_counts[r]);
    ws += uint64_t(h_recv_words[r]);
  }
  if (hs != n_recv || (ws && !d_recv_words)) {
    set_error("smash_dedup_owner: per-source counts do not add up to n_recv");
    return SMASH_ERR_ARG;
  }
  base[world] = hs;
  base[65 + world] = ws;
  p->last = s;
  if (!n_recv) return SMASH_OK;
  if (n_recv > p->oslot_cap) {
    SMASH_HIP(hipStreamSynchronize(s));
    if (p->d_oslot) SMASH_HIP(hipFree(p->d_oslot));
    p->oslot_cap = n_recv + n_recv / 4 + 1024;
    SMASH_HIP(hipMalloc(reinterpret_cast<void **>(&p->d_oslot), 8 * p->oslot_cap));
  }
  SMASH_HIP(hipMemcpyAsync(p->d_recv_base, base, 8 * 2 * 65, hipMemcpyHostToDevice, s));
  SMASH_HIP(hipEventRecord(p->ev_base, s));
  const uint64_t epoch = next_epoch(p);
  k_owner_claim<<<grid_for(n_recv, kB, 8192), kB, 0, s>>>(
      d_recv, d_recv_words, p->d_recv_base, world, n_recv, p->d_table, p->table_mask, p->d_arena,
      epoch, p->d_oslot, p->d_stats, p->hash_mask);
  SMASH_HIP(hipGetLastError());
  k_owner_decide<<<grid_for((n_recv + kDecGroups - 1) / kDecGroups, kB, 8192), kB, 0, s>>>(
      d_recv, d_recv_words, p->d_recv_base, world, n_recv, p->d_table, p->d_arena, p->arena_cap,
      p->d_arena_top, epoch, p->d_oslot, d_flags, p->d_stats, p->hash_mask);
  SMASH_HIP(hipGetLastError());
  return SMASH_OK;
}

extern "C" int smash_phase_import(smash_pipeline *p, const uint8_t *d_flags_back,
                                  void *stream) {
  if (!p) return SMASH_ERR_ARG;
  hipStream_t s = static_cast<hipStream_t>(stream);
  p->last = s;
  if (p->n_export)
    k_import<<<grid_for(p->n_export, kB, 1u << 30), kB, 0, s>>>(d_flags_back, p->d_send_q,
                                                               p->n_export, p->d_keep);
  if (p->n_pairs)
    k_import_stats<<<grid_for(p->n_pairs, kB, 1u << 30), kB, 0, s>>>(p->d_keep, p->d_nk,
                                                                    p->n_pairs, p->d_stats);
  SMASH_HIP(hipGetLastError());
  return SMASH_OK;
}

extern "C" int smash_pipeline_error(smash_pipeline *p, void *stream, int32_t *err) {
  if (!p || !err) return SMASH_ERR_ARG;
  SMASH_HIP(hipSetDevice(p->device));
  hipStream_t s = static_cast<hipStream_t>(stream);
  SMASH_HIP(hipMemcpyAsync(p->h_owner + 192, p->d_stats + S_ERR, 8, hipMemcpyDeviceToHost, s));
  SMASH_HIP(hipStreamSynchronize(s));
  *err = int32_t(p->h_owner[192]);
  return SMASH_OK;
}

extern "C" int smash_pipeline_stats(smash_pipeline *p, smash_stats *o) {
  if (!p || !o) return SMASH_ERR_ARG;
  SMASH_HIP(hipSetDevice(p->device));
  if (p->last) SMASH_HIP(hipStreamSynchronize(p->last));
  SMASH_HIP(hipDeviceSynchronize());
  if (int rc = probe_check(p->ix)) return rc;
  unsigned long long rows[kStatWords], st[S_N] = {0};
  SMASH_HIP(hipMemcpy(rows, p->d_stats, sizeof(rows), hipMemcpyDeviceToHost));
  for (uint32_t r = 0; r < kStatStripes; ++r)
    for (int k = 0; k < S_N; ++k)
      if (k != S_ERR) st[k] += rows[r * kStatStride + k];
  st[S_ERR] = rows[S_ERR];
  o->pairs = st[S_PAIRS];
  o->key_pairs = st[S_KEYPAIRS];
  o->dupe_pairs = st[S_DUPEPAIRS];
  o->positions = st[S_POS];
  o->dups = st[S_DUPS];
  o->kept = st[S_KEPT];
  o->matches = st[S_MATCHES];
  o->error = int32_t(st[S_ERR]);
  return SMASH_OK;
}

extern "C" int smash_pipeline_peek(smash_pipeline *p, int32_t *h_nk, uint8_t *h_keep,
                                   uint64_t *h_hits, uint64_t *h_hash) {
  if (!p) return SMASH_ERR_ARG;
  SMASH_HIP(hipSetDevice(p->device));
  SMASH_HIP(hipDeviceSynchronize());
  const uint64_t n = p->n_pairs;
  if (!n) return SMASH_OK;
  if (h_nk) SMASH_HIP(hipMemcpy(h_nk, p->d_nk, 4 * n, hipMemcpyDeviceToHost));
  if (h_keep) SMASH_HIP(hipMemcpy(h_keep, p->d_keep, n, hipMemcpyDeviceToHost));
  if (h_hits) {
    const uint64_t W = 2 * uint64_t(p->slots);
    SMASH_HIP(hipMemcpy(h_hits, p->d_hits, 8 * n * W, hipMemcpyDeviceToHost));
    std::vector<int32_t> nk(n);
    std::vector<uint64_t> head(n * smash::kHitHead);
    SMASH_HIP(hipMemcpy(nk.data(), p->d_nk, 4 * n, hipMemcpyDeviceToHost));
    SMASH_HIP(hipMemcpy(head.data(), p->d_hhead, 8 * n * smash::kHitHead, hipMemcpyDeviceToHost));
    for (uint64_t q = 0; q < n; ++q)
      if (nk[q] > 0 && nk[q] <= int32_t(smash::kHitHead))
        std::memcpy(h_hits + q * W, head.data() + q * smash::kHitHead, 8 * size_t(nk[q]));
  }
  if (h_hash) SMASH_HIP(hipMemcpy(h_hash, p->d_hash, 16 * n, hipMemcpyDeviceToHost));
  return SMASH_OK;
}

extern "C" int smash_pipeline_reserve_keys(smash_pipeline *p, uint64_t keys, void *stream) {
  if (!p) return SMASH_ERR_ARG;
  uint64_t slots = 0, words = 0;
  key_set_geometry(keys, p->max_pairs, &slots, &words);
  slots = std::max<uint64_t>(slots, p->table_mask + 1);
  words = std::max<uint64_t>(words, p->arena_cap);
  if (slots <= p->table_mask + 1 && words <= p->arena_cap) return SMASH_OK;
  SMASH_HIP(hipSetDevice(p->device));
  SMASH_HIP(hipDeviceSynchronize());
  unsigned long long top = 0;
  SMASH_HIP(hipMemcpy(&top, p->d_arena_top, 8, hipMemcpyDeviceToHost));
  uint64_t *t = nullptr, *a = nullptr;
  if (hipMalloc(reinterpret_cast<void **>(&t), 16 * slots) != hipSuccess ||
      hipMalloc(reinterpret_cast<void **>(&a), 8 * words) != hipSuccess) {
    (void)hipFree(t);
    set_error("smash_pipeline_reserve_keys: out of device memory for " + std::to_string(keys) +
              " keys");
    return SMASH_ERR_NOMEM;
  }
  hipStream_t s = static_cast<hipStream_t>(stream);
  SMASH_HIP(hipMemsetAsync(t, 0, 16 * slots, s));
  if (top) {
    SMASH_HIP(hipMemcpyAsync(a, p->d_arena, 8 * std::min<uint64_t>(top, p->arena_cap),
                             hipMemcpyDeviceToDevice, s));
    const uint64_t old_slots = p->table_mask + 1;
    k_rehash<<<grid_for(old_slots, 256, 1u << 16), 256, 0, s>>>(p->d_table, old_slots, t, slots - 1);
    SMASH_HIP(hipGetLastError());
  }
  SMASH_HIP(hipStreamSynchronize(s));
  SMASH_HIP(hipFree(p->d_table));
  SMASH_HIP(hipFree(p->d_arena));
  p->d_table = t;
  p->d_arena = a;
  p->table_mask = slots - 1;
  p->arena_cap = words;
  return SMASH_OK;
}

namespace smash {
int ensure_keys(smash_pipeline *p, uint64_t n_next, hipStream_t s) {
  const uint64_t need = p->keys_bound + n_next, cap = smash_pipeline_key_capacity(p);
  if (need <= cap) return SMASH_OK;
  return smash_pipeline_reserve_keys(p, std::max(need, 2 * cap), s);
}
}

extern "C" uint64_t smash_pipeline_key_capacity(const smash_pipeline *p) {
  return p ? std::min<uint64_t>((p->table_mask + 1) / 2, p->arena_cap / 16) : 0;
}

extern "C" int smash_pipeline_map_hints(const smash_pipeline *p) { return p && p->mhint ? 1 : 0; }

extern "C" int smash_pipeline_reset_ex(smash_pipeline *p, uint32_t flags, void *stream) {
  if (!p || (flags & ~uint32_t(SMASH_RESET_KEEP_SEARCH))) return SMASH_ERR_ARG;
  hipStream_t s = static_cast<hipStream_t>(stream);
  SMASH_HIP(hipSetDevice(p->device));
  SMASH_HIP(hipMemsetAsync(p->d_table, 0, 16 * (p->table_mask + 1), s));
  SMASH_HIP(hipMemsetAsync(p->d_arena_top, 0, 8, s));
  p->keys_bound = 0;
  SMASH_HIP(hipMemsetAsync(p->d_stats, 0, 8 * kStatWords, s));
  k_reset_prev<<<1, 1, 0, s>>>(p->d_prev);
  SMASH_HIP(hipGetLastError());
  if (!(flags & SMASH_RESET_KEEP_SEARCH))
    for (int k = 0; k < 2; ++k) {
      p->searched[k] = false;
      p->pref_reads[k] = nullptr;
      p->pref_n[k] = 0;
    }
  return SMASH_OK;
}

extern "C" int smash_pipeline_reset(smash_pipeline *p, void *stream) {
  return smash_pipeline_reset_ex(p, 0, stream);
}

extern "C" int smash_pipeline_var_len(smash_pipeline *p, int on) {
  if (!p) return SMASH_ERR_ARG;
  if (p->searched[0] || p->searched[1]) {
    set_error("smash_pipeline_var_len: a look-ahead search is pending");
    return SMASH_ERR_ARG;
  }
  p->var_len = on != 0;
  return SMASH_OK;
}

extern "C" int smash_pipeline_peek_lens(smash_pipeline *p, uint16_t *h_lens) {
  if (!p || !h_lens) return SMASH_ERR_ARG;
  SMASH_HIP(hipSetDevice(p->device));
  SMASH_HIP(hipDeviceSynchronize());
  const uint64_t n = p->n_pairs;
  if (!n) return SMASH_OK;
  if (!p->d_lens) {
    std::fill(h_lens, h_lens + 2 * n, uint16_t(p->read_len));
    return SMASH_OK;
  }
  SMASH_HIP(hipMemcpy(h_lens, p->d_lens, 2 * 2 * n, hipMemcpyDeviceToHost));
  return SMASH_OK;
}

extern "C" int smash_pipeline_peek_matches(smash_pipeline *p, uint64_t *h_words, uint32_t *h_n) {
  if (!p || !h_words || !h_n) return SMASH_ERR_ARG;
  SMASH_HIP(hipSetDevice(p->device));
  SMASH_HIP(hipDeviceSynchronize());
  const uint64_t n = p->n_pairs;
  if (!n) return SMASH_OK;
  SMASH_HIP(hipMemcpy(h_words, p->d_match, 8 * 2 * n * p->slots, hipMemcpyDeviceToHost));
  SMASH_HIP(hipMemcpy(h_n, p->d_nmatch, 4 * 2 * n, hipMemcpyDeviceToHost));
  return SMASH_OK;
}

extern "C" int smash_pipeline_reads_resident(smash_pipeline *p, int on) {
  if (!p) return SMASH_ERR_ARG;
  p->reads_resident = on != 0;
  return SMASH_OK;
}

extern "C" int smash_pipeline_profile(smash_pipeline *p, int enable) {
  if (!p) return SMASH_ERR_ARG;
  p->prof = enable != 0;
  p->n_ev = 0;
  p->prof_reads = 0;
  return SMASH_OK;
}

extern "C" int smash_pipeline_profile_read(smash_pipeline *p, double *search_ms,
                                           uint64_t *launches, uint64_t *reads) {
  if (!p) return SMASH_ERR_ARG;
  SMASH_HIP(hipSetDevice(p->device));
  double ms = 0;
  for (uint64_t i = 0; i < p->n_ev; ++i) {
    SMASH_HIP(hipEventSynchronize(p->ev[2 * i + 1]));
    float t = 0;
    SMASH_HIP(hipEventElapsedTime(&t, p->ev[2 * i], p->ev[2 * i + 1]));
    ms += t;
  }
  if (search_ms) *search_ms = ms;
  if (launches) *launches = p->n_ev;
  if (reads) *reads = p->prof_reads;
  return SMASH_OK;
}

extern "C" int smash_pipeline_profile_intervals(smash_pipeline *p, double *h_ms, uint64_t cap,
                                                uint64_t *n) {
  if (!p || !n || (cap && !h_ms)) return SMASH_ERR_ARG;
  SMASH_HIP(hipSetDevice(p->device));
  *n = p->n_ev;
  for (uint64_t i = 0; i < p->n_ev && i < cap; ++i) {
    SMASH_HIP(hipEventSynchronize(p->ev[2 * i + 1]));
    float a = 0, b = 0;
    SMASH_HIP(hipEventElapsedTime(&a, p->ev[0], p->ev[2 * i]));
    SMASH_HIP(hipEventElapsedTime(&b, p->ev[0], p->ev[2 * i + 1]));
    h_ms[2 * i] = a;
    h_ms[2 * i + 1] = b;
  }
  return SMASH_OK;
}

extern "C" int smash_pipeline_profile_active(smash_pipeline *p, double *active_ms) {
  if (!p || !active_ms) return SMASH_ERR_ARG;
  SMASH_HIP(hipSetDevice(p->device));
  std::vector<std::pair<double, double>> iv;
  for (uint64_t i = 0; i < p->n_ev; ++i) {
    SMASH_HIP(hipEventSynchronize(p->ev[2 * i + 1]));
    float a = 0, b = 0;
    SMASH_HIP(hipEventElapsedTime(&a, p->ev[0], p->ev[2 * i]));
    SMASH_HIP(hipEventElapsedTime(&b, p->ev[0], p->ev[2 * i + 1]));
    iv.emplace_back(a, b);
  }
  std::sort(iv.begin(), iv.end());
  double tot = 0, cs = 0, ce = -1e300;
  for (const auto &x : iv) {
    if (x.first > ce) {
      if (ce > cs) tot += ce - cs;
      cs = x.first;
      ce = x.second;
    } else if (x.second > ce) {
      ce = x.second;
    }
  }
  if (!iv.empty() && ce > cs) tot += ce - cs;
  *active_ms = tot;
  return SMASH_OK;
}

extern "C" int smash_pipeline_positions(smash_pipeline *p, int64_t *h_pos0, int64_t *h_abspos,
                                        uint64_t cap, uint64_t *n_out) {
  if (!p || !n_out) return SMASH_ERR_ARG;
  SMASH_HIP(hipSetDevice(p->device));
  if (p->pos_dirty && p->n_pairs) {
    SMASH_HIP(ensure_positions(p));
    k_emit<<<grid_for(p->n_pairs, kB, 1u << 30), kB, 0, p->last>>>(
        p->d_keep, p->d_nk, hit_rows(p), p->d_posoff, p->n_pairs, p->d_chrom_off,
        p->d_pos0, p->d_abs);
    SMASH_HIP(hipGetLastError());
    p->pos_dirty = false;
  }
  if (p->last) SMASH_HIP(hipStreamSynchronize(p->last));
  uint32_t n = 0;
  if (p->n_pairs)
    SMASH_HIP(hipMemcpy(&n, p->d_posoff + p->n_pairs, 4, hipMemcpyDeviceToHost));
  *n_out = n;
  const uint64_t k = n < cap ? n : cap;
  if (k && h_pos0) SMASH_HIP(hipMemcpy(h_pos0, p->d_pos0, 8 * k, hipMemcpyDeviceToHost));
  if (k && h_abspos) SMASH_HIP(hipMemcpy(h_abspos, p->d_abs, 8 * k, hipMemcpyDeviceToHost));
  return SMASH_OK;
}

extern "C" int smash_bin_positions(const int64_t *d_pos0, const int64_t *d_abspos, uint64_t n,
                                   int64_t prev_pos0, const int64_t *d_bin_starts,
                                   uint32_t nbins, uint64_t *d_counts, uint64_t *h_stats,
                                   void *stream) {
  if ((n && (!d_pos0 || !d_abspos)) || !d_bin_starts || nbins == 0 || !d_counts || !h_stats) {
    set_error("smash_bin_positions: bad arguments");
    return SMASH_ERR_ARG;
  }
  hipStream_t s = static_cast<hipStream_t>(stream);
  uint64_t *scratch = nullptr;
  SMASH_HIP(hipMallocAsync(reinterpret_cast<void **>(&scratch), 8 * (2 + S_N), s));
  SMASH_HIP(hipMemsetAsync(scratch, 0, 8 * (2 + S_N), s));
  int rc = SMASH_OK;
  for (uint64_t b = 0; b < n && rc == SMASH_OK; b += (1ull << 30)) {
    const uint64_t m = n - b < (1ull << 30) ? n - b : (1ull << 30);
    const uint32_t m32 = uint32_t(m);
    const bool first = b == 0;
    if (hipMemcpyAsync(scratch, &m32, 4, hipMemcpyHostToDevice, s) != hipSuccess ||
        hipMemcpyAsync(scratch + 1, first ? static_cast<const void *>(&prev_pos0) : &d_pos0[b - 1],
                       8, first ? hipMemcpyHostToDevice : hipMemcpyDeviceToDevice,
                       s) != hipSuccess) {
      rc = SMASH_ERR_HIP;
      break;
    }
    k_bin<<<2048, kB, 0, s>>>(d_pos0 + b, d_abspos + b, reinterpret_cast<const uint32_t *>(scratch),
                              reinterpret_cast<const int64_t *>(scratch + 1), d_bin_starts, nbins,
                              nullptr, 0, 0,
                              reinterpret_cast<unsigned long long *>(d_counts),
                              reinterpret_cast<unsigned long long *>(scratch + 2));
    if (hipGetLastError() != hipSuccess) rc = SMASH_ERR_HIP;
    if (hipStreamSynchronize(s) != hipSuccess) rc = SMASH_ERR_HIP;
  }
  uint64_t st[S_N] = {0};
  if (rc == SMASH_OK && hipMemcpyAsync(st, scratch + 2, sizeof(st), hipMemcpyDeviceToHost, s) != hipSuccess)
    rc = SMASH_ERR_HIP;
  if (hipStreamSynchronize(s) != hipSuccess) rc = SMASH_ERR_HIP;
  (void)hipFree(scratch);
  if (rc != SMASH_OK) {
    set_error("smash_bin_positions: HIP error");
    return rc;
  }
  h_stats[0] += st[S_POS];
  h_stats[1] += st[S_DUPS];
  h_stats[2] += st[S_KEPT];
  return SMASH_OK;
}
```

Before: 505.8 million reads/s.

## Keep dedup keys in persistent hit-head rows instead of copying into arena

Dedup keys whose hit count fits in the head row are no longer copied into the arena. Table entries now reference a persistent global row index (row_base + q), and a match against an earlier batch compares directly against the stored head rows. The decide kernel skips the wave scan and the arena atomic when no lane needs an arena record. Last-position computation moves into the post-processing kernels, so decide no longer rescans hit rows. In exchange, per-pair nk and head rows must be kept for all keys across batches, which adds memory and device-to-device copies when capacity grows.

```diff
diff --git a/smash-paper_amd/csrc/keyset.hpp b/smash-paper_amd/csrc/keyset.hpp
--- a/smash-paper_amd/csrc/keyset.hpp
+++ b/smash-paper_amd/csrc/keyset.hpp
@@ -5,6 +5,13 @@
 
 constexpr int kRefShift = 40;
 constexpr uint64_t kRefPub = 1ull << 39;
+struct KeyStore {
+  uint64_t *table;
+  uint64_t mask;
+  const uint64_t *arena;
+  const uint64_t *rows;
+  const int32_t *row_nk;
+};
 struct KeyRef {
   const uint64_t *w;
   uint32_t nk;
@@ -22,6 +29,14 @@
   if (a.lo != b.lo || a.nk != b.nk) return false;
   for (uint32_t i = 0; i < a.nk; ++i)
     if (a.w[i] != b.w[i]) return false;
+  return true;
+}
+
+__device__ bool same_key(const KeyStore &st, uint64_t g, const KeyRef &k) {
+  if (k.nk > kHitHead || st.row_nk[g] != int32_t(k.nk)) return false;
+  const uint64_t *r = st.rows + g * kHitHead;
+  for (uint32_t i = 0; i < k.nk; ++i)
+    if (r[i] != k.w[i]) return false;
   return true;
 }
 
@@ -93,6 +108,15 @@
   const uint64_t *hash;
   HitRows hits;
   uint8_t *contest;
+  uint64_t row_base;
+  static __device__ __forceinline__ bool in_arena(int32_t m) { return m > int32_t(kHitHead); }
+  __device__ __forceinline__ unsigned long long claim(uint64_t q, uint64_t) const {
+    return row_base + q + 1;
+  }
+  __device__ __forceinline__ bool claimed(unsigned long long ref, uint64_t, uint64_t &q2) const {
+    q2 = ref - 1 - row_base;
+    return (ref >> (kRefShift - 1)) == 0 && ref > row_base;
+  }
   __device__ __forceinline__ int32_t count(uint64_t q) const { return nk[q]; }
   __device__ __forceinline__ KeyRef key(uint64_t q, uint64_t *hi = nullptr) const {
     if (hi) *hi = hash[2 * q];
@@ -106,6 +130,15 @@
   const uint64_t *recv, *words, *base;
   int world;
   uint64_t hmask;
+  static __device__ __forceinline__ bool in_arena(int32_t) { return true; }
+  __device__ __forceinline__ unsigned long long claim(uint64_t j, uint64_t epoch) const {
+    return (epoch << kRefShift) | (j + 1);
+  }
+  __device__ __forceinline__ bool claimed(unsigned long long ref, uint64_t epoch,
+                                          uint64_t &j2) const {
+    j2 = (ref & (kRefPub - 1)) - 1;
+    return !(ref & kRefPub) && (ref >> kRefShift) == epoch;
+  }
   __device__ __forceinline__ int32_t count(uint64_t j) const {
     return int32_t(recv[kHdrWords * j] >> 40);
   }
@@ -122,12 +155,13 @@
 };
 
 template <class Src>
-__device__ __forceinline__ uint64_t claim_key(const Src &src, uint64_t j, uint64_t *table,
-                                              uint64_t mask, const uint64_t *arena,
+__device__ __forceinline__ uint64_t claim_key(const Src &src, uint64_t j, const KeyStore &st,
                                               uint64_t epoch, int32_t &err) {
+  uint64_t *const table = st.table;
+  const uint64_t mask = st.mask;
   uint64_t hi = 0;
   const KeyRef me = src.key(j, &hi);
-  const unsigned long long mine = (epoch << kRefShift) | (j + 1);
+  const unsigned long long mine = src.claim(j, epoch);
   uint64_t res = kSlotNone;
   uint64_t i = key_home(hi, mask);
   uint32_t waits = 0;
@@ -154,18 +188,23 @@
         }
         continue;
       }
+      uint64_t j2 = 0;
       if (ref & kRefPub) {
         if ((ref >> kRefShift) != epoch &&
-            same_key(arena + ((ref & (kRefPub - 1)) - 1), me)) {
+            same_key(st.arena + ((ref & (kRefPub - 1)) - 1), me)) {
           res = kSlotOld;
           break;
         }
-      } else if ((ref >> kRefShift) == epoch) {
-        const uint64_t j2 = (ref & (kRefPub - 1)) - 1;
+      } else if (src.claimed(ref, epoch, j2)) {
         if (same_key(me, src.key(j2))) {
           if constexpr (Src::kMarks) src.contest[j2] = 1;
           atomicMin(sr, mine);
           res = i;
+          break;
+        }
+      } else if ((ref >> kRefShift) == 0) {
+        if (same_key(st, ref - 1, me)) {
+          res = kSlotOld;
           break;
         }
       }
@@ -188,8 +227,8 @@
   for (uint64_t c0 = (uint64_t(blockIdx.x) * blockDim.x + (threadIdx.x & ~63u)) * kDecGroups;
        c0 < n; c0 += stride * kDecGroups) {
     bool wins[kDecGroups];
-    uint32_t needs[kDecGroups], incls[kDecGroups], tots[kDecGroups];
-    uint32_t sum = 0;
+    uint32_t needs[kDecGroups];
+    bool rec = false;
 #pragma unroll
     for (uint32_t g = 0; g < kDecGroups; ++g) {
       const uint64_t j = c0 + 64 * g + lane;
@@ -205,104 +244,102 @@
           const unsigned long long ref = __hip_atomic_load(
               reinterpret_cast<unsigned long long *>(&table[2 * (sl & ~kSlotIns) + 1]),
               __ATOMIC_RELAXED, __HIP_MEMORY_SCOPE_AGENT);
-          win = ref == ((epoch << kRefShift) | (j + 1));
+          win = ref == src.claim(j, epoch);
         }
       }
       wins[g] = win;
-      needs[g] = win ? 2u + uint32_t(m) : 0u;
-      incls[g] = wave_incl(needs[g], tots[g]);
-      sum += tots[g];
-    }
-    unsigned long long wbase = 0;
-    if (lane == 63 && sum) wbase = atomicAdd(arena_top, (unsigned long long)sum);
-    wbase = __shfl(wbase, 63, 64);
+      needs[g] = win && Src::in_arena(m) ? 2u + uint32_t(m) : 0u;
+      rec = rec || needs[g];
+    }
+    if (__any(rec)) {
+      uint32_t incls[kDecGroups], tots[kDecGroups];
+      uint32_t sum = 0;
+#pragma unroll
+      for (uint32_t g = 0; g < kDecGroups; ++g) {
+        incls[g] = wave_incl(needs[g], tots[g]);
+        sum += tots[g];
+      }
+      unsigned long long wbase = 0;
+      if (lane == 63) wbase = atomicAdd(arena_top, (unsigned long long)sum);
+      wbase = __shfl(wbase, 63, 64);
+#pragma unroll
+      for (uint32_t g = 0; g < kDecGroups; ++g) {
+        const uint64_t j = c0 + 64 * g + lane;
+        const uint32_t need = needs[g], incl = incls[g], total = tots[g];
+        const uint64_t off = uint64_t(wbase) + incl - need;
+        wbase += total;
+        const bool ok = need && off + need <= arena_cap;
+        KeyRef me{nullptr, 0u, 0ull};
+        if (need) me = src.key(j);
+        wave_fill_records(arena, off, incl, total, ok, me.lo, me.nk, me.w);
+        if (need) {
+          if (!ok) {
+            full = true;
+          } else {
+            __hip_atomic_store(
+                reinterpret_cast<unsigned long long *>(&table[2 * (slot_of[j] & ~kSlotIns) + 1]),
+                (unsigned long long)((epoch << kRefShift) | kRefPub | (off + 1)),
+                __ATOMIC_RELAXED, __HIP_MEMORY_SCOPE_AGENT);
+          }
+        }
+      }
+    }
 #pragma unroll
     for (uint32_t g = 0; g < kDecGroups; ++g) {
       const uint64_t j = c0 + 64 * g + lane;
-      const bool win = wins[g];
-      const uint32_t need = needs[g], incl = incls[g], total = tots[g];
-      const uint64_t off = uint64_t(wbase) + incl - need;
-      wbase += total;
-      const bool ok = win && off + need <= arena_cap;
-      KeyRef me{nullptr, 0u, 0ull};
-      if (win) me = src.key(j);
-      wave_fill_records(arena, off, incl, total, ok, me.lo, me.nk, me.w);
-      if (win) {
-        if (!ok) {
-          full = true;
-        } else {
-          __hip_atomic_store(
-              reinterpret_cast<unsigned long long *>(&table[2 * (slot_of[j] & ~kSlotIns) + 1]),
-              (unsigned long long)((epoch << kRefShift) | kRefPub | (off + 1)), __ATOMIC_RELAXED,
-              __HIP_MEMORY_SCOPE_AGENT);
-        }
-      }
-      if (j < n) item(j, win);
+      if (j < n) item(j, wins[g]);
     }
   }
   return full;
 }
 
 __global__ void k_dedup_claim(const int32_t *__restrict__ nk, const uint64_t *__restrict__ hash,
-                              HitRows hits, uint64_t n,
-                              uint64_t *table, uint64_t mask, const uint64_t *arena,
+                              HitRows hits, uint64_t n, uint64_t row_base, KeyStore st,
                               uint64_t epoch, uint64_t *slot_of, uint8_t *contest,
                               unsigned long long *stats) {
   SMASH_BESIDE_SEARCH();
-  const PairKeys src{nk, hash, hits, contest};
+  const PairKeys src{nk, hash, hits, contest, row_base};
   const uint64_t stride = uint64_t(gridDim.x) * blockDim.x;
   int32_t err = 0;
   for (uint64_t q = uint64_t(blockIdx.x) * blockDim.x + threadIdx.x; q < n; q += stride)
-    if (nk[q] >= 0) slot_of[q] = claim_key(src, q, table, mask, arena, epoch, err);
+    if (nk[q] >= 0) slot_of[q] = claim_key(src, q, st, epoch, err);
   if (err) atomicCAS(&stats[S_ERR], 0ull, (unsigned long long)(unsigned)err);
 }
 
 __global__ void k_dedup_decide(const int32_t *__restrict__ nk, const uint64_t *__restrict__ hash,
-                               HitRows hits,
-                               const uint32_t *__restrict__ nmajor,
-                               const int64_t *__restrict__ chrom_off, uint64_t n,
-                               uint64_t *table, uint64_t *arena, uint64_t arena_cap,
-                               unsigned long long *arena_top, uint64_t epoch,
+                               HitRows hits, const uint32_t *__restrict__ nmajor, uint64_t n,
+                               uint64_t row_base, uint64_t *table, uint64_t *arena,
+                               uint64_t arena_cap, unsigned long long *arena_top, uint64_t epoch,
                                const uint64_t *__restrict__ slot_of,
                                const uint8_t *__restrict__ contest, uint8_t *keep,
                                uint32_t *cnt, int64_t *lp, unsigned long long *stats) {
   SMASH_BESIDE_SEARCH();
-  const PairKeys src{nk, hash, hits, const_cast<uint8_t *>(contest)};
+  const PairKeys src{nk, hash, hits, const_cast<uint8_t *>(contest), row_base};
   unsigned long long kp = 0, dp = 0;
   const bool full = decide_keys(
       src, n, table, arena, arena_cap, arena_top, epoch, slot_of,
       [&](uint64_t q, bool win) __attribute__((always_inline)) {
-        const int32_t m = nk[q];
-        if (m >= 0) {
+        if (nk[q] >= 0) {
           ++kp;
-          dp += win ? 0 : 1;
+          if (!win) {
+            ++dp;
+            lp[q] = -1;
+          }
         }
         keep[q] = win ? 1 : 0;
-        const uint32_t c = win ? nmajor[q] : 0;
-        cnt[q] = c;
-        int64_t last = -1;
-        if (c) {
-          const uint64_t *h = hits.row(q, m);
-          for (int32_t j = m - 1; j >= 0; --j)
-            if (chrom_off[uint32_t(h[j] >> 48)] >= 0) {
-              last = int64_t(h[j] & 0xFFFFFFFFFFFFull);
-              break;
-            }
-        }
-        lp[q] = last;
+        cnt[q] = win ? nmajor[q] : 0;
       });
   wave_stats(stats, S_KEYPAIRS, kp, S_DUPEPAIRS, dp, full ? SMASH_ERR_NOMEM : 0);
 }
 
 __global__ void k_owner_claim(const uint64_t *recv, const uint64_t *words, const uint64_t *base,
-                              int world, uint64_t n, uint64_t *table, uint64_t mask,
-                              const uint64_t *arena, uint64_t epoch, uint64_t *slot_of,
-                              unsigned long long *stats, uint64_t hmask) {
+                              int world, uint64_t n, KeyStore st, uint64_t epoch,
+                              uint64_t *slot_of, unsigned long long *stats, uint64_t hmask) {
   const RecvKeys src{recv, words, base, world, hmask};
   const uint64_t stride = uint64_t(gridDim.x) * blockDim.x;
   int32_t err = 0;
   for (uint64_t j = uint64_t(blockIdx.x) * blockDim.x + threadIdx.x; j < n; j += stride)
-    slot_of[j] = claim_key(src, j, table, mask, arena, epoch, err);
+    slot_of[j] = claim_key(src, j, st, epoch, err);
   if (err) atomicCAS(&stats[S_ERR], 0ull, (unsigned long long)(unsigned)err);
 }
 
@@ -322,14 +359,15 @@
 }
 }
 
-static void key_set_geometry(uint64_t keys, uint64_t max_pairs, uint64_t *slots,
-                             uint64_t *arena_words) {
-  const uint64_t cap = 2 * std::max<uint64_t>(keys, max_pairs);
+struct KeySetGeometry {
+  uint64_t slots, rows, arena_words, owner_arena_words;
+};
+static KeySetGeometry key_set_geometry(uint64_t keys, uint64_t max_pairs) {
+  const uint64_t k = std::max<uint64_t>(keys, max_pairs);
   uint64_t pw = 1;
-  while (pw < cap) pw <<= 1;
-  *slots = pw;
-  *arena_words = std::min<uint64_t>(16 * std::max<uint64_t>(keys, max_pairs) + (1u << 20),
-                                    smash::kRefPub - 2);
+  while (pw < 2 * k) pw <<= 1;
+  return KeySetGeometry{pw, k, k + (1u << 20),
+                        std::min<uint64_t>(16 * k + (1u << 20), smash::kRefPub - 2)};
 }
 
 static uint64_t next_epoch(smash_pipeline *p) {
diff --git a/smash-paper_amd/csrc/pipeline.hip b/smash-paper_amd/csrc/pipeline.hip
--- a/smash-paper_amd/csrc/pipeline.hip
+++ b/smash-paper_amd/csrc/pipeline.hip
@@ -59,6 +59,9 @@
   uint32_t *d_nmajor = nullptr;
   uint64_t *d_hits = nullptr;
   uint64_t *d_hhead = nullptr;
+  uint64_t row_cap = 0;
+  uint64_t row_base = 0;
+  uint64_t row_next = 0;
   uint64_t *d_hash = nullptr;
   uint8_t *d_keep = nullptr;
   uint64_t *d_slot = nullptr;
@@ -77,6 +80,7 @@
   uint64_t *d_arena = nullptr;
   uint64_t arena_cap = 0;
   unsigned long long *d_arena_top = nullptr;
+  bool owner_arena = false;
   uint64_t keys_bound = 0;
   uint64_t epoch = 0;
   uint32_t *d_posoff = nullptr;
@@ -272,8 +276,8 @@
 __device__ __noinline__ void post_pair(const PostCfg &c, const uint64_t *__restrict__ match,
                                        const uint32_t *__restrict__ nmatch, uint64_t q,
                                        int32_t *nk_out, uint32_t *nmajor_out,
-                                       HitRows hits_out, uint64_t *hash_out, int32_t &err,
-                                       unsigned long long &nm, uint8_t *ws) {
+                                       HitRows hits_out, uint64_t *hash_out, int64_t *lp_out,
+                                       int32_t &err, unsigned long long &nm, uint8_t *ws) {
   {
     Aln *a = reinterpret_cast<Aln *>(ws);
     Hit *h1 = reinterpret_cast<Hit *>(ws + uint64_t(c.slots) * sizeof(Aln));
@@ -298,6 +302,7 @@
     uint64_t *ho = hits_out.full + q * (2 * uint64_t(c.slots));
     int32_t nk = -1;
     uint32_t nmaj = 0;
+    int64_t lastp = -1;
     uint64_t hh = 0x9E3779B97F4A7C15ull, hl = 0xD1B54A32D192ED03ull;
     if (m1 > 0 || m2 > 0) {
       nk = 0;
@@ -306,7 +311,10 @@
         const uint64_t w = (uint64_t(tid) << 48) ^ uint64_t(pos);
         hh = mix64(hh ^ w) + 0x632BE59BD9B4E019ull;
         hl = mix64(hl + w * 0x9E3779B97F4A7C15ull) ^ (hl >> 29);
-        if (c.chrom_off[tid] >= 0) ++nmaj;
+        if (c.chrom_off[tid] >= 0) {
+          ++nmaj;
+          lastp = int64_t(uint64_t(pos) & 0xFFFFFFFFFFFFull);
+        }
       };
       for (int i = 0; i < m1; ++i) put(h1[i].tid, h1[i].pos);
       for (int b = 0; b < m2; ++b) {
@@ -325,6 +333,7 @@
     }
     nk_out[q] = nk;
     nmajor_out[q] = nmaj;
+    lp_out[q] = lastp;
     hash_out[2 * q] = hh;
     hash_out[2 * q + 1] = hl;
   }
@@ -365,8 +374,8 @@
                                              uint64_t n_pairs, const uint32_t *list,
                                              const uint32_t *n_list, int32_t *nk_out,
                                              uint32_t *nmajor_out, HitRows hits_out,
-                                             uint64_t *hash_out, unsigned long long *stats,
-                                             uint8_t *ws) {
+                                             uint64_t *hash_out, int64_t *lp_out,
+                                             unsigned long long *stats, uint8_t *ws) {
   SMASH_BESIDE_SEARCH();
   int32_t err = 0;
   unsigned long long nm = 0, np = 0;
@@ -375,8 +384,8 @@
   const uint64_t n = list ? *n_list : n_pairs;
   for (uint64_t i = t; i < n; i += uint64_t(gridDim.x) * blockDim.x) {
     unsigned long long m = 0;
-    post_pair<VAR>(c, match, nmatch, list ? list[i] : i, nk_out, nmajor_out, hits_out, hash_out, err,
-              m, my);
+    post_pair<VAR>(c, match, nmatch, list ? list[i] : i, nk_out, nmajor_out, hits_out, hash_out,
+                   lp_out, err, m, my);
     nm += m;
     ++np;
   }
@@ -596,7 +605,7 @@
                                                   uint32_t *up_list, uint32_t *up_n,
                                                   int32_t *nk_out, uint32_t *nmajor_out,
                                                   HitRows hits_out, uint64_t *hash_out,
-                                                  unsigned long long *stats) {
+                                                  int64_t *lp_out, unsigned long long *stats) {
   SMASH_BESIDE_SEARCH();
   const uint64_t *sp = c.startpos;
   const uint64_t n = list ? *n_list : n_pairs;
@@ -622,6 +631,7 @@
                               : hits_out.full + q * (2 * uint64_t(c.slots));
       int32_t nk = -1;
       uint32_t nmaj = 0;
+      int64_t lastp = -1;
       uint64_t hh = 0x9E3779B97F4A7C15ull, hl = 0xD1B54A32D192ED03ull;
       bool any = false;
 #pragma unroll
@@ -635,7 +645,10 @@
           const uint64_t x = (uint64_t(tid) << 48) ^ uint64_t(pos);
           hh = mix64(hh ^ x) + 0x632BE59BD9B4E019ull;
           hl = mix64(hl + x * 0x9E3779B97F4A7C15ull) ^ (hl >> 29);
-          if (c.chrom_off[tid] >= 0) ++nmaj;
+          if (c.chrom_off[tid] >= 0) {
+            ++nmaj;
+            lastp = pos;
+          }
         };
 #pragma unroll
         for (int i = 0; i < CAP; ++i)
@@ -660,6 +673,7 @@
       }
       nk_out[q] = nk;
       nmajor_out[q] = nmaj;
+      lp_out[q] = lastp;
       hash_out[2 * q] = hh;
       hash_out[2 * q + 1] = hl;
     }
@@ -1114,7 +1128,10 @@
   return c;
 }
 
-HitRows hit_rows(const smash_pipeline *p) { return HitRows{p->d_hhead, p->d_hits, p->slots}; }
+HitRows hit_rows(const smash_pipeline *p) {
+  return HitRows{p->d_hhead + p->row_base * kHitHead, p->d_hits, p->slots};
+}
+int32_t *pair_nk(const smash_pipeline *p) { return p->d_nk + p->row_base; }
 
 }
 }
@@ -1254,10 +1271,12 @@
     SMASH_HIPX(hipEventSynchronize(p->ev_done));
     p->d_match = p->d_match_s[0];
     p->d_nmatch = p->d_nmatch_s[0];
-    p->d_nk = dalloc<int32_t>(P);
+    const KeySetGeometry geo = key_set_geometry(cfg->dedup_capacity, P);
+    p->row_cap = geo.rows;
+    p->d_nk = dalloc<int32_t>(p->row_cap);
     p->d_nmajor = dalloc<uint32_t>(P);
     p->d_hits = dalloc<uint64_t>(P * 2 * p->slots);
-    p->d_hhead = dalloc<uint64_t>(P * smash::kHitHead);
+    p->d_hhead = dalloc<uint64_t>(p->row_cap * smash::kHitHead);
     p->d_hash = dalloc<uint64_t>(2 * P);
     p->d_keep = dalloc<uint8_t>(P);
     {
@@ -1270,8 +1289,10 @@
     }
     p->d_posoff = dalloc<uint32_t>(P + 1);
     p->d_cnt = dalloc<uint32_t>(P);
-    uint64_t pw = 0;
-    key_set_geometry(cfg->dedup_capacity, P, &pw, &p->arena_cap);
+    const uint64_t pw = geo.slots;
+    p->arena_cap = geo.arena_words;
+    if (const char *aw = getenv("SMASH_KEY_ARENA_WORDS"))
+      if (*aw) p->arena_cap = std::max<uint64_t>(1, std::strtoull(aw, nullptr, 10));
     p->table_mask = pw - 1;
     p->d_table = dalloc<uint64_t>(2 * pw);
     SMASH_HIPX(hipMemset(p->d_table, 0, 16 * pw));
@@ -1440,19 +1461,21 @@
     const PostCfg pc = post_cfg(p);
     k_post_fast<8, VAR><<<grid_for(n_pairs, kB, 1u << 30), kB, 0, s>>>(
         pc, p->d_match, p->d_nmatch, n_pairs, nullptr, nullptr, std::min(8u, p->post_cap),
-        p->d_l16 + 1, p->d_l16, p->d_nk, p->d_nmajor, hit_rows(p), p->d_hash, p->d_stats);
+        p->d_l16 + 1, p->d_l16, pair_nk(p), p->d_nmajor, hit_rows(p), p->d_hash, p->d_lp,
+        p->d_stats);
     SMASH_HIP(hipGetLastError());
     k_post_fast<FCAP, VAR><<<grid_for(n_pairs, kB, 1024), kB, 0, s>>>(
         pc, p->d_match, p->d_nmatch, n_pairs, p->d_l16 + 1, p->d_l16, p->post_cap,
-        p->d_fb + 1, p->d_fb, p->d_nk, p->d_nmajor, hit_rows(p), p->d_hash, p->d_stats);
+        p->d_fb + 1, p->d_fb, pair_nk(p), p->d_nmajor, hit_rows(p), p->d_hash, p->d_lp,
+        p->d_stats);
     SMASH_HIP(hipGetLastError());
     k_post<VAR><<<kPostBlocks, kB, 0, s>>>(post_cfg(p), p->d_match, p->d_nmatch, n_pairs,
-                                           p->d_fb + 1, p->d_fb, p->d_nk, p->d_nmajor, hit_rows(p),
-                                           p->d_hash, p->d_stats, p->d_post_ws);
+                                           p->d_fb + 1, p->d_fb, pair_nk(p), p->d_nmajor, hit_rows(p),
+                                           p->d_hash, p->d_lp, p->d_stats, p->d_post_ws);
   } else {
     k_post<VAR><<<kPostBlocks, kB, 0, s>>>(post_cfg(p), p->d_match, p->d_nmatch, n_pairs, nullptr,
-                                           nullptr, p->d_nk, p->d_nmajor, hit_rows(p), p->d_hash,
-                                           p->d_stats, p->d_post_ws);
+                                           nullptr, pair_nk(p), p->d_nmajor, hit_rows(p), p->d_hash,
+                                           p->d_lp, p->d_stats, p->d_post_ws);
   }
   SMASH_HIP(hipGetLastError());
   return SMASH_OK;
@@ -1465,6 +1488,11 @@
   if (rc) return rc;
   if (d_next && (rc = check_pipe(p, n_next))) return rc;
   p->last = s;
+  p->row_base = p->row_next;
+  p->n_pairs = 0;
+  if (p->row_base + n_pairs > p->row_cap &&
+      (rc = smash_pipeline_reserve_keys(p, std::max(p->row_base + n_pairs, 2 * p->row_cap), s)))
+    return rc;
   p->n_pairs = n_pairs;
   if (!n_pairs) return SMASH_OK;
   SMASH_HIP(hipSetDevice(p->device));
@@ -1523,21 +1551,29 @@
   return search_into(p, k, d_reads, n_pairs, p->ev_in);
 }
 
+static int grow_key_set(smash_pipeline *p, uint64_t slots, uint64_t rows, uint64_t words,
+                        hipStream_t s);
+
+static KeyStore key_store(const smash_pipeline *p) {
+  return KeyStore{p->d_table, p->table_mask, p->d_arena, p->d_hhead, p->d_nk};
+}
+
 static int dedup_local(smash_pipeline *p, hipStream_t s) {
   const uint64_t n = p->n_pairs;
   if (!n) return SMASH_OK;
   const uint64_t epoch = next_epoch(p);
   SMASH_HIP(hipMemsetAsync(p->d_contest, 0, n, s));
-  k_dedup_claim<<<grid_for(n, kB, 8192), kB, 0, s>>>(p->d_nk, p->d_hash, hit_rows(p), n,
-                                                     p->d_table, p->table_mask, p->d_arena, epoch,
-                                                     p->d_slot, p->d_contest, p->d_stats);
+  k_dedup_claim<<<grid_for(n, kB, 8192), kB, 0, s>>>(pair_nk(p), p->d_hash, hit_rows(p), n,
+                                                     p->row_base, key_store(p), epoch, p->d_slot,
+                                                     p->d_contest, p->d_stats);
   SMASH_HIP(hipGetLastError());
   k_dedup_decide<<<grid_for((n + kDecGroups - 1) / kDecGroups, kB, 8192), kB, 0, s>>>(
-      p->d_nk, p->d_hash, hit_rows(p), p->d_nmajor, p->d_chrom_off, n, p->d_table,
-      p->d_arena, p->arena_cap, p->d_arena_top, epoch, p->d_slot, p->d_contest, p->d_keep,
-      p->d_cnt, p->d_lp, p->d_stats);
+      pair_nk(p), p->d_hash, hit_rows(p), p->d_nmajor, n, p->row_base, p->d_table, p->d_arena,
+      p->arena_cap, p->d_arena_top, epoch, p->d_slot, p->d_contest, p->d_keep, p->d_cnt,
+      p->d_lp, p->d_stats);
   SMASH_HIP(hipGetLastError());
   p->cnt_ready = true;
+  p->row_next = p->row_base + n;
   return SMASH_OK;
 }
 
@@ -1548,7 +1584,7 @@
   const uint64_t n = p->n_pairs;
   if (n) {
     if (!p->cnt_ready)
-      k_count_last<<<grid_for(n, kB, 1u << 30), kB, 0, s>>>(p->d_keep, p->d_nmajor, p->d_nk,
+      k_count_last<<<grid_for(n, kB, 1u << 30), kB, 0, s>>>(p->d_keep, p->d_nmajor, pair_nk(p),
                                                            hit_rows(p), p->d_chrom_off,
                                                            n, p->d_cnt, p->d_lp);
     const uint64_t ntile = (n + kScanTile - 1) / kScanTile;
@@ -1578,14 +1614,14 @@
     const unsigned gx = unsigned(std::min<uint64_t>(kBinBlocks, (n + 1023) / 1024));
     const dim3 grid(gx, parts);
     k_emit_bin_lds<<<grid, 1024, 0, s>>>(
-        p->d_keep, p->d_nk, hit_rows(p), p->d_chrom_off, p->d_lps, n, prev, p->d_bins,
+        p->d_keep, pair_nk(p), hit_rows(p), p->d_chrom_off, p->d_lps, n, prev, p->d_bins,
         p->nbins, p->d_cell, p->ncell, p->cshift, reinterpret_cast<unsigned long long *>(d_counts),
         p->d_stats, part, p->bin_flush, p->d_binpart);
     k_bin_reduce<<<grid_for(p->nbins, kB, 1024), kB, 0, s>>>(
         p->d_binpart, gx, p->nbins, reinterpret_cast<unsigned long long *>(d_counts));
   } else if (n) {
     k_emit_bin<<<grid_for(n, kB, 8192), kB, 0, s>>>(
-        p->d_keep, p->d_nk, hit_rows(p), p->d_chrom_off, p->d_lps, n, prev, p->d_bins,
+        p->d_keep, pair_nk(p), hit_rows(p), p->d_chrom_off, p->d_lps, n, prev, p->d_bins,
         p->nbins, p->d_cell, p->ncell, p->cshift, reinterpret_cast<unsigned long long *>(d_counts),
         p->d_stats);
   }
@@ -1808,7 +1844,7 @@
   unsigned long long *cnt = p->h_owner;
   std::fill(cnt, cnt + 128, 0ull);
   if (n) {
-    k_export_count<<<nblk, kB, 0, s>>>(p->d_nk, p->d_hash, n, world, nblk, p->d_bcnt);
+    k_export_count<<<nblk, kB, 0, s>>>(pair_nk(p), p->d_hash, n, world, nblk, p->d_bcnt);
     size_t tb = p->scan_temp_bytes;
     SMASH_HIP(hipcub::DeviceScan::ExclusiveSum(p->d_scan_temp, tb, p->d_bcnt, p->d_boff,
                                                uint64_t(world) * nblk, s));
@@ -1831,7 +1867,7 @@
     SMASH_HIP(hipMalloc(&p->d_send_words, 8 * p->send_words_cap));
   }
   if (n)
-    k_export_fill<<<nblk, kB, 0, s>>>(p->d_nk, p->d_hash, hit_rows(p), n, world, nblk,
+    k_export_fill<<<nblk, kB, 0, s>>>(pair_nk(p), p->d_hash, hit_rows(p), n, world, nblk,
                                       p->d_boff, p->d_send_hdr, p->d_send_words, p->d_send_q);
   SMASH_HIP(hipGetLastError());
   *d_send = p->d_send_hdr;
@@ -1873,12 +1909,17 @@
     p->oslot_cap = n_recv + n_recv / 4 + 1024;
     SMASH_HIP(hipMalloc(reinterpret_cast<void **>(&p->d_oslot), 8 * p->oslot_cap));
   }
+  if (!p->owner_arena) {
+    p->owner_arena = true;
+    if (int rc = grow_key_set(p, 0, 0, key_set_geometry(p->row_cap, 0).owner_arena_words, s))
+      return rc;
+  }
   SMASH_HIP(hipMemcpyAsync(p->d_recv_base, base, 8 * 2 * 65, hipMemcpyHostToDevice, s));
   SMASH_HIP(hipEventRecord(p->ev_base, s));
   const uint64_t epoch = next_epoch(p);
   k_owner_claim<<<grid_for(n_recv, kB, 8192), kB, 0, s>>>(
-      d_recv, d_recv_words, p->d_recv_base, world, n_recv, p->d_table, p->table_mask, p->d_arena,
-      epoch, p->d_oslot, p->d_stats, p->hash_mask);
+      d_recv, d_recv_words, p->d_recv_base, world, n_recv, key_store(p), epoch, p->d_oslot,
+      p->d_stats, p->hash_mask);
   SMASH_HIP(hipGetLastError());
   k_owner_decide<<<grid_for((n_recv + kDecGroups - 1) / kDecGroups, kB, 8192), kB, 0, s>>>(
       d_recv, d_recv_words, p->d_recv_base, world, n_recv, p->d_table, p->d_arena, p->arena_cap,
@@ -1896,7 +1937,7 @@
     k_import<<<grid_for(p->n_export, kB, 1u << 30), kB, 0, s>>>(d_flags_back, p->d_send_q,
                                                                p->n_export, p->d_keep);
   if (p->n_pairs)
-    k_import_stats<<<grid_for(p->n_pairs, kB, 1u << 30), kB, 0, s>>>(p->d_keep, p->d_nk,
+    k_import_stats<<<grid_for(p->n_pairs, kB, 1u << 30), kB, 0, s>>>(p->d_keep, pair_nk(p),
                                                                     p->n_pairs, p->d_stats);
   SMASH_HIP(hipGetLastError());
   return SMASH_OK;
@@ -1942,15 +1983,16 @@
   SMASH_HIP(hipDeviceSynchronize());
   const uint64_t n = p->n_pairs;
   if (!n) return SMASH_OK;
-  if (h_nk) SMASH_HIP(hipMemcpy(h_nk, p->d_nk, 4 * n, hipMemcpyDeviceToHost));
+  if (h_nk) SMASH_HIP(hipMemcpy(h_nk, pair_nk(p), 4 * n, hipMemcpyDeviceToHost));
   if (h_keep) SMASH_HIP(hipMemcpy(h_keep, p->d_keep, n, hipMemcpyDeviceToHost));
   if (h_hits) {
     const uint64_t W = 2 * uint64_t(p->slots);
     SMASH_HIP(hipMemcpy(h_hits, p->d_hits, 8 * n * W, hipMemcpyDeviceToHost));
     std::vector<int32_t> nk(n);
     std::vector<uint64_t> head(n * smash::kHitHead);
-    SMASH_HIP(hipMemcpy(nk.data(), p->d_nk, 4 * n, hipMemcpyDeviceToHost));
-    SMASH_HIP(hipMemcpy(head.data(), p->d_hhead, 8 * n * smash::kHitHead, hipMemcpyDeviceToHost));
+    SMASH_HIP(hipMemcpy(nk.data(), pair_nk(p), 4 * n, hipMemcpyDeviceToHost));
+    SMASH_HIP(hipMemcpy(head.data(), hit_rows(p).head, 8 * n * smash::kHitHead,
+                        hipMemcpyDeviceToHost));
     for (uint64_t q = 0; q < n; ++q)
       if (nk[q] > 0 && nk[q] <= int32_t(smash::kHitHead))
         std::memcpy(h_hits + q * W, head.data() + q * smash::kHitHead, 8 * size_t(nk[q]));
@@ -1959,42 +2001,71 @@
   return SMASH_OK;
 }
 
-extern "C" int smash_pipeline_reserve_keys(smash_pipeline *p, uint64_t keys, void *stream) {
-  if (!p) return SMASH_ERR_ARG;
-  uint64_t slots = 0, words = 0;
-  key_set_geometry(keys, p->max_pairs, &slots, &words);
-  slots = std::max<uint64_t>(slots, p->table_mask + 1);
-  words = std::max<uint64_t>(words, p->arena_cap);
-  if (slots <= p->table_mask + 1 && words <= p->arena_cap) return SMASH_OK;
+static int grow_key_set(smash_pipeline *p, uint64_t slots, uint64_t rows, uint64_t words,
+                        hipStream_t s) {
+  const uint64_t old_slots = p->table_mask + 1;
+  slots = std::max(slots, old_slots);
+  rows = std::max(rows, p->row_cap);
+  words = std::max(words, p->arena_cap);
+  if (slots == old_slots && rows == p->row_cap && words == p->arena_cap) return SMASH_OK;
   SMASH_HIP(hipSetDevice(p->device));
   SMASH_HIP(hipDeviceSynchronize());
   unsigned long long top = 0;
   SMASH_HIP(hipMemcpy(&top, p->d_arena_top, 8, hipMemcpyDeviceToHost));
-  uint64_t *t = nullptr, *a = nullptr;
-  if (hipMalloc(reinterpret_cast<void **>(&t), 16 * slots) != hipSuccess ||
-      hipMalloc(reinterpret_cast<void **>(&a), 8 * words) != hipSuccess) {
+  uint64_t *t = nullptr, *a = nullptr, *h = nullptr;
+  int32_t *k = nullptr;
+  if ((slots > old_slots && hipMalloc(reinterpret_cast<void **>(&t), 16 * slots) != hipSuccess) ||
+      (words > p->arena_cap && hipMalloc(reinterpret_cast<void **>(&a), 8 * words) != hipSuccess) ||
+      (rows > p->row_cap &&
+       (hipMalloc(reinterpret_cast<void **>(&h), 8 * rows * smash::kHitHead) != hipSuccess ||
+        hipMalloc(reinterpret_cast<void **>(&k), 4 * rows) != hipSuccess))) {
     (void)hipFree(t);
-    set_error("smash_pipeline_reserve_keys: out of device memory for " + std::to_string(keys) +
+    (void)hipFree(a);
+    (void)hipFree(h);
+    (void)hipFree(k);
+    set_error("smash_pipeline_reserve_keys: out of device memory for " + std::to_string(rows) +
               " keys");
     return SMASH_ERR_NOMEM;
   }
-  hipStream_t s = static_cast<hipStream_t>(stream);
-  SMASH_HIP(hipMemsetAsync(t, 0, 16 * slots, s));
-  if (top) {
+  if (t) {
+    SMASH_HIP(hipMemsetAsync(t, 0, 16 * slots, s));
+    k_rehash<<<grid_for(old_slots, 256, 1u << 16), 256, 0, s>>>(p->d_table, old_slots, t, slots - 1);
+    SMASH_HIP(hipGetLastError());
+  }
+  if (a && top)
     SMASH_HIP(hipMemcpyAsync(a, p->d_arena, 8 * std::min<uint64_t>(top, p->arena_cap),
                              hipMemcpyDeviceToDevice, s));
-    const uint64_t old_slots = p->table_mask + 1;
-    k_rehash<<<grid_for(old_slots, 256, 1u << 16), 256, 0, s>>>(p->d_table, old_slots, t, slots - 1);
-    SMASH_HIP(hipGetLastError());
+  const uint64_t held = std::min(p->row_cap, std::max(p->row_next, p->row_base + p->n_pairs));
+  if (h && held) {
+    SMASH_HIP(hipMemcpyAsync(h, p->d_hhead, 8 * held * smash::kHitHead, hipMemcpyDeviceToDevice, s));
+    SMASH_HIP(hipMemcpyAsync(k, p->d_nk, 4 * held, hipMemcpyDeviceToDevice, s));
   }
   SMASH_HIP(hipStreamSynchronize(s));
-  SMASH_HIP(hipFree(p->d_table));
-  SMASH_HIP(hipFree(p->d_arena));
-  p->d_table = t;
-  p->d_arena = a;
-  p->table_mask = slots - 1;
-  p->arena_cap = words;
-  return SMASH_OK;
+  if (t) {
+    SMASH_HIP(hipFree(p->d_table));
+    p->d_table = t;
+    p->table_mask = slots - 1;
+  }
+  if (a) {
+    SMASH_HIP(hipFree(p->d_arena));
+    p->d_arena = a;
+    p->arena_cap = words;
+  }
+  if (h) {
+    SMASH_HIP(hipFree(p->d_hhead));
+    SMASH_HIP(hipFree(p->d_nk));
+    p->d_hhead = h;
+    p->d_nk = k;
+    p->row_cap = rows;
+  }
+  return SMASH_OK;
+}
+
+extern "C" int smash_pipeline_reserve_keys(smash_pipeline *p, uint64_t keys, void *stream) {
+  if (!p) return SMASH_ERR_ARG;
+  const KeySetGeometry g = key_set_geometry(keys, p->max_pairs);
+  return grow_key_set(p, g.slots, g.rows, p->owner_arena ? g.owner_arena_words : g.arena_words,
+                      static_cast<hipStream_t>(stream));
 }
 
 namespace smash {
@@ -2006,7 +2077,9 @@
 }
 
 extern "C" uint64_t smash_pipeline_key_capacity(const smash_pipeline *p) {
-  return p ? std::min<uint64_t>((p->table_mask + 1) / 2, p->arena_cap / 16) : 0;
+  if (!p) return 0;
+  const uint64_t cap = std::min<uint64_t>((p->table_mask + 1) / 2, p->row_cap);
+  return p->owner_arena ? std::min<uint64_t>(cap, p->arena_cap / 16) : cap;
 }
 
 extern "C" int smash_pipeline_map_hints(const smash_pipeline *p) { return p && p->mhint ? 1 : 0; }
@@ -2018,6 +2091,7 @@
   SMASH_HIP(hipMemsetAsync(p->d_table, 0, 16 * (p->table_mask + 1), s));
   SMASH_HIP(hipMemsetAsync(p->d_arena_top, 0, 8, s));
   p->keys_bound = 0;
+  p->row_base = p->row_next = 0;
   SMASH_HIP(hipMemsetAsync(p->d_stats, 0, 8 * kStatWords, s));
   k_reset_prev<<<1, 1, 0, s>>>(p->d_prev);
   SMASH_HIP(hipGetLastError());
@@ -2150,7 +2224,7 @@
   if (p->pos_dirty && p->n_pairs) {
     SMASH_HIP(ensure_positions(p));
     k_emit<<<grid_for(p->n_pairs, kB, 1u << 30), kB, 0, p->last>>>(
-        p->d_keep, p->d_nk, hit_rows(p), p->d_posoff, p->n_pairs, p->d_chrom_off,
+        p->d_keep, pair_nk(p), hit_rows(p), p->d_posoff, p->n_pairs, p->d_chrom_off,
         p->d_pos0, p->d_abs);
     SMASH_HIP(hipGetLastError());
     p->pos_dirty = false;
```

New measurement: 517.8 million reads/s, median of 6. 2.4% higher.
